# cheshmi/parsy_bench

Measured on AMD Instinct MI355X. Metric: Cholesky factorizations/sec (+ SpTRSV solves/sec), SuiteSparse SPD set, higher is better.
Workload: dtype f64; 1 GPU; flan-class stand-in (BASELINE.json configs[2] when flan: Flan_1565): grid (116, 116, 116) 27-point stencil, geometric nested dissection; n=1560896, nnz_A_lower=21491316, nsuper=81191, nnz_L=2044454227, xsize=2421483055, etree_levels=17, launches_per_factorization=357, parallelism=1 GPU

## Files before the change

### include/parsy_amd.h

```cpp
#ifndef PARSY_AMD_H
#define PARSY_AMD_H

#include <stdbool.h>
#include <stddef.h>
#include <stdint.h>

#ifdef __cplusplus
extern "C" {
#endif


bool cholesky_left_par_05(int n, int* c, int* r, double* values, size_t* lC, int* lR,
                          size_t* Li_ptr, double* lValues, int* blockSet, int supNo,
                          double* timing, int* aTree, int* cT, int* rT, int* col2Sup,
                          int nLevels, int* levelPtr, int* levelSet, int nPar, int* parPtr,
                          int* partition, int chunk, int threads, int super_max, int col_max,
                          double* nodCost);

bool cholesky_left_par_05_prune(int n, int* c, int* r, double* values, size_t* lC, int* lR,
                                size_t* Li_ptr, double* lValues, int* blockSet, int supNo,
                                double* timing, int* prunePtr, int* pruneSet, int nLevels,
                                int* levelPtr, int* levelSet, int nPar, int* parPtr, int* partition,
                                int chunk, int threads, int super_max, int col_max, double* nodCost);

bool cholesky_left_par_waveFront(int n, int* c, int* r, double* values, size_t* lC, int* lR,
                                 size_t* Li_ptr, double* lValues, int* blockSet, int supNo,
                                 double* timing, int* aTree, int* cT, int* rT, int* col2Sup,
                                 int nLevels, int* levelPtr, int* levelSet, int chunk,
                                 int threads, int super_max, int col_max);

int blockedLsolve(int n, size_t* Lp, int* Li, double* Lx, int NNZ, size_t* Li_ptr,
                  int* col2sup, int* sup2col, int supNo, double* x);
int leveledBlockedLsolve(int n, size_t* Lp, int* Li, double* Lx, int NNZ, size_t* Li_ptr,
                         int* col2sup, int* sup2col, int supNo, double* x, int levels,
                         int* levelPtr, int* levelSet, int chunk);
int H2LeveledBlockedLsolve(int n, size_t* Lp, int* Li, double* Lx, int NNZ, size_t* Li_ptr,
                           int* col2sup, int* sup2col, int supNo, double* x, int levels,
                           int* levelPtr, int* levelSet, int parts, int* parPtr,
                           int* partition, int chunk);
int H2LeveledBlockedLsolve_Peeled(int n, size_t* Lp, int* Li, double* Lx, int NNZ,
                                  size_t* Li_ptr, int* col2sup, int* sup2col, int supNo,
                                  double* x, int levels, int* levelPtr, int* levelSet,
                                  int parts, int* parPtr, int* partition, int chunk,
                                  int threads);

void parsy_dropin_reset(void);


typedef struct parsy_plan parsy_plan;

typedef struct parsy_plan_info {
    int32_t n, nsuper, nlevels, max_width, max_rows;
    int32_t n_small, n_big;
    int32_t chol_launches;
    int32_t solve_launches;
    int64_t nnzA, ssize, xsize, nnzL;
    int64_t n_updates;
    int64_t relpos_len;
    int64_t device_bytes;
    double flops_stored;
    double update_flops;
    double reread_bytes;
    double inner_flops;
    double tile_update_flops;
    double big_flops;
    int64_t big_entries;
    int32_t big_tasks;
    int32_t n_pieces;
    int32_t chol_levels;
    int32_t piece_width, big_min_k;
    int32_t chol_subtrees, chol_subtree_supernodes;
    int32_t solve_subtrees, solve_subtree_supernodes;
    int32_t backsolve_launches;
    int32_t dense_tasks;
    double dense_flops;
    int64_t dense_entries;
    int32_t solve_one;
    int32_t solve_one_blocks;
    int32_t sub_mrhs_trees;
    int32_t sub_mrhs_slots;
    int32_t sub_mrhs_tiers;
    int32_t sub_mrhs_cover_level;
    int64_t dense_strip_entries;
} parsy_plan_info;

parsy_plan* parsy_plan_create(int n, int supNo, const int* blockSet, const size_t* lC,
                              const size_t* Li_ptr, const int* lR, const int* aTree,
                              const int* col2Sup, const int* cT, const int* rT, const int* c,
                              const int* r, int device);
void parsy_plan_destroy(parsy_plan* plan);
int parsy_plan_get_info(const parsy_plan* plan, parsy_plan_info* info);

int parsy_plan_set_active(parsy_plan* plan, const uint8_t* mask);
long long parsy_plan_chain_check(const parsy_plan* plan, int slots);
long long parsy_plan_check(const parsy_plan* plan);

int parsy_factor_device(parsy_plan* plan, const double* d_values, double* d_lValues,
                        void* stream);
#define PARSY_FACTOR_NO_INIT 1
int parsy_factor_device_ex(parsy_plan* plan, const double* d_values, double* d_lValues,
                           void* stream, int flags);
int parsy_factor_status(parsy_plan* plan);

int parsy_factor_begin(parsy_plan* plan, const double* d_values, double* d_lValues, void* stream, int flags);
int parsy_factor_level(parsy_plan* plan, int level, double* d_lValues, void* stream);
int parsy_factor_end(parsy_plan* plan, void* stream);
int parsy_plan_pieces(const parsy_plan* plan, int32_t* supernode, int32_t* level, int32_t* col0, int32_t* width,
                      int32_t* rows, int64_t* value_begin, int64_t* value_end);
int parsy_plan_set_active_pieces(parsy_plan* plan, const uint8_t* piece_mask);

typedef struct parsy_dist parsy_dist;
typedef struct parsy_dist_info {
    int32_t nranks, nlevels, n_pieces, n_subtrees, n_root_pieces, n_messages;
    int64_t exchange_elements;
    double total_cost, root_cost;
    double max_rank_cost;
    double lockstep_cost;
} parsy_dist_info;
parsy_dist* parsy_dist_create(const parsy_plan* plan, int nranks, int block);
void parsy_dist_destroy(parsy_dist* dist);
int parsy_dist_get_info(const parsy_dist* dist, parsy_dist_info* info);
int parsy_dist_get(const parsy_dist* dist, int32_t* owner, uint8_t* in_subtree, double* rank_cost,
                   double* level_cost);
int parsy_dist_level_messages(const parsy_dist* dist, int level);
int parsy_dist_message(const parsy_dist* dist, int level, int index, int32_t* src, int32_t* dst, int64_t* nseg,
                       int64_t* total, const int64_t** off, const int32_t** len, const int64_t** packed);
long long parsy_dist_check(const parsy_plan* plan, const parsy_dist* dist);

int parsy_solve_device(parsy_plan* plan, const double* d_lValues, double* d_x, int nrhs,
                       int ldx, void* stream);

int parsy_solve_status(parsy_plan* plan);

int parsy_backsolve_device(parsy_plan* plan, const double* d_lValues, double* d_x, int nrhs, int ldx,
                           void* stream);
int parsy_plan_solve_levels(const parsy_plan* plan, int32_t* level);
#define PARSY_SOLVE_FIRST 1
#define PARSY_SOLVE_LAST 2
#define PARSY_SOLVE_BACKWARD 4
int parsy_solve_levels_device(parsy_plan* plan, const double* d_lValues, double* d_x, int nrhs, int ldx, void* stream,
                              int level_begin, int level_end, int flags);
int parsy_rhs_ones_device(parsy_plan* plan, const double* d_lValues, double* d_b, void* stream);
int parsy_copy_segments_device(double* d_dst, const double* d_src, const int64_t* d_dst_off,
                               const int64_t* d_src_off, const int32_t* d_len, int64_t nseg, void* stream);
int parsy_solve2_host(parsy_plan* plan, const double* lValues, double* x, int nrhs, int ldx,
                      int forward, double* seconds);

int parsy_plan_set_perm(parsy_plan* plan, const int* perm);
int parsy_residual_device(parsy_plan* plan, const double* d_values, const double* d_x, int ldx, const double* d_b,
                          int ldb, double* d_r, int ldr, int nrhs, double* berr, void* stream);
int parsy_solve_spd_device(parsy_plan* plan, const double* d_values, const double* d_lValues, const double* d_b,
                           int ldb, double* d_x, int ldx, int nrhs, int max_steps, int32_t* steps, double* berr,
                           void* stream);
int parsy_solve_spd_host(parsy_plan* plan, const double* values, const double* lValues, const double* b, int ldb,
                         double* x, int ldx, int nrhs, int max_steps, int32_t* steps, double* berr, double* seconds);

typedef struct parsy_selinv_info {
    int32_t levels;
    int32_t block_columns;
    int32_t tiled_block_columns;
    int32_t launches;
    double  flops;
    int64_t device_bytes;
} parsy_selinv_info;
int parsy_selinv_get_info(parsy_plan* plan, parsy_selinv_info* info);
long long parsy_selinv_check(const parsy_plan* plan);
int parsy_selinv_device(parsy_plan* plan, const double* d_lValues, double* d_z, void* stream);
int parsy_inverse_diag_device(parsy_plan* plan, const double* d_z, double* d_diag, void* stream);
int parsy_selinv_host(parsy_plan* plan, const double* lValues, double* z, double* diag, double* seconds);
int parsy_logdet_device(parsy_plan* plan, const double* d_lValues, double* logdet, void* stream);

int parsy_factor_host(parsy_plan* plan, const double* values, double* lValues, double* seconds);
int parsy_solve_host(parsy_plan* plan, const double* lValues, double* x, int nrhs, int ldx,
                     double* seconds);

double parsy_last_factor_ms(parsy_plan* plan);
double parsy_last_solve_ms(parsy_plan* plan);

#define PARSY_PROFILE_KINDS 10
int parsy_plan_profile(parsy_plan* plan, int enable);
int parsy_plan_profile_collect(parsy_plan* plan);
int parsy_plan_profile_get(parsy_plan* plan, double* kind_ms, int* kind_launches, int* runs);
int parsy_plan_profile_levels(parsy_plan* plan, double* main_ms, double* side_ms);

const char* parsy_last_error(void);

int parsy_device_count(void);

int parsy_debug_kernel_count(void);
const char* parsy_debug_kernel_name(int k);
unsigned long long parsy_debug_kernel_launches(int k);
void parsy_debug_kernel_reset(void);


typedef struct parsy_symbolic parsy_symbolic;

typedef struct parsy_symbolic_view {
    int32_t n, nsuper, nlevels, maxSupWid, maxCol;
    int64_t ssize, xsize, nnzL, nnzA, n_updates;
    double flops_colcount, flops_stored;
    const int* Perm;
    const int* Parent;
    const int* ColCount;
    const int* super;
    const int* col2Sup;
    const int* sParent;
    const size_t* p;
    const size_t* i_ptr;
    const int* s;
    const int* A1p; const int* A1i;
    const int* A2p; const int* A2i; const double* A2x;
    const int* A2src;
    const int* levelPtr;
    const int* levelSet;
    const int64_t* updPtr;
    const int* updSn; const int* updLb; const int* updUb;
} parsy_symbolic_view;

parsy_symbolic* parsy_analyze(int n, const int* Ap, const int* Ai, const double* Ax,
                              const int* perm, const int* nrelax, const double* zrelax);
void parsy_symbolic_free(parsy_symbolic* sym);
int parsy_symbolic_get(const parsy_symbolic* sym, parsy_symbolic_view* view);
parsy_plan* parsy_plan_from_symbolic(const parsy_symbolic* sym, int device);


int64_t parsy_grid_spd_lower(int nx, int ny, int nz, int stencil, double shift, int* Ap,
                             int* Ai, double* Ax);
int parsy_grid_nested_dissection(int nx, int ny, int nz, int leaf, int* perm);
int parsy_order_nd(int n, const int* Ap, const int* Ai, int leaf, int* perm);


typedef struct parsy_mg parsy_mg;
parsy_mg* parsy_mg_create(const parsy_symbolic* sym, int nranks, const int* devices, int block);
void parsy_mg_destroy(parsy_mg* mg);
int parsy_mg_set_values(parsy_mg* mg, const double* values);
int parsy_mg_factor(parsy_mg* mg, double* seconds);
int parsy_mg_profile(parsy_mg* mg, double* main_ms, double* side_ms, double* copy_ms);
int parsy_mg_rank_ms(parsy_mg* mg, double* rank_ms);
int parsy_mg_gather_host(parsy_mg* mg, double* lValues);
const parsy_dist* parsy_mg_dist(const parsy_mg* mg);
parsy_plan* parsy_mg_plan(parsy_mg* mg, int rank);

#ifdef __cplusplus
}
#endif
#endif
```

### parsy_bench_amd/_native.py

```python
from __future__ import annotations

import ctypes as C
import os
from pathlib import Path

import numpy as np

_PKG = Path(__file__).resolve().parent
_LIB_PATH = Path(os.environ["PARSY_LIB"]) if os.environ.get("PARSY_LIB") else _PKG / "libparsy_amd.so"
_lib = None

c_int_p = C.POINTER(C.c_int)
c_dbl_p = C.POINTER(C.c_double)
c_size_p = C.POINTER(C.c_size_t)
c_i64_p = C.POINTER(C.c_int64)


class SymbolicView(C.Structure):
    _fields_ = [
        ("n", C.c_int32), ("nsuper", C.c_int32), ("nlevels", C.c_int32),
        ("maxSupWid", C.c_int32), ("maxCol", C.c_int32),
        ("ssize", C.c_int64), ("xsize", C.c_int64), ("nnzL", C.c_int64),
        ("nnzA", C.c_int64), ("n_updates", C.c_int64),
        ("flops_colcount", C.c_double), ("flops_stored", C.c_double),
        ("Perm", c_int_p), ("Parent", c_int_p), ("ColCount", c_int_p),
        ("super", c_int_p), ("col2Sup", c_int_p), ("sParent", c_int_p),
        ("p", c_size_p), ("i_ptr", c_size_p), ("s", c_int_p),
        ("A1p", c_int_p), ("A1i", c_int_p),
        ("A2p", c_int_p), ("A2i", c_int_p), ("A2x", c_dbl_p), ("A2src", c_int_p),
        ("levelPtr", c_int_p), ("levelSet", c_int_p),
        ("updPtr", c_i64_p), ("updSn", c_int_p), ("updLb", c_int_p), ("updUb", c_int_p),
    ]


class PlanInfo(C.Structure):
    _fields_ = [
        ("n", C.c_int32), ("nsuper", C.c_int32), ("nlevels", C.c_int32),
        ("max_width", C.c_int32), ("max_rows", C.c_int32),
        ("n_small", C.c_int32), ("n_big", C.c_int32),
        ("chol_launches", C.c_int32), ("solve_launches", C.c_int32),
        ("nnzA", C.c_int64), ("ssize", C.c_int64), ("xsize", C.c_int64), ("nnzL", C.c_int64),
        ("n_updates", C.c_int64), ("relpos_len", C.c_int64), ("device_bytes", C.c_int64),
        ("flops_stored", C.c_double), ("update_flops", C.c_double), ("reread_bytes", C.c_double),
        ("inner_flops", C.c_double), ("tile_update_flops", C.c_double),
        ("big_flops", C.c_double), ("big_entries", C.c_int64), ("big_tasks", C.c_int32),
        ("n_pieces", C.c_int32), ("chol_levels", C.c_int32), ("piece_width", C.c_int32),
        ("big_min_k", C.c_int32),
        ("chol_subtrees", C.c_int32), ("chol_subtree_supernodes", C.c_int32),
        ("solve_subtrees", C.c_int32), ("solve_subtree_supernodes", C.c_int32),
        ("backsolve_launches", C.c_int32), ("dense_tasks", C.c_int32),
        ("dense_flops", C.c_double), ("dense_entries", C.c_int64),
        ("solve_one", C.c_int32), ("solve_one_blocks", C.c_int32),
        ("sub_mrhs_trees", C.c_int32), ("sub_mrhs_slots", C.c_int32),
        ("sub_mrhs_tiers", C.c_int32), ("sub_mrhs_cover_level", C.c_int32),
        ("dense_strip_entries", C.c_int64),
    ]

    def as_dict(self):
        return {k: getattr(self, k) for k, _ in self._fields_}


EXPORTED_SYMBOLS = [
    "cholesky_left_par_05", "cholesky_left_par_05_prune", "cholesky_left_par_waveFront", "blockedLsolve",
    "leveledBlockedLsolve", "H2LeveledBlockedLsolve", "H2LeveledBlockedLsolve_Peeled",
    "parsy_dropin_reset", "parsy_plan_create", "parsy_plan_destroy", "parsy_plan_get_info",
    "parsy_plan_set_active", "parsy_plan_chain_check", "parsy_factor_device", "parsy_factor_status", "parsy_solve_device",
    "parsy_factor_host", "parsy_solve_host", "parsy_last_factor_ms", "parsy_last_solve_ms",
    "parsy_last_error", "parsy_device_count", "parsy_analyze", "parsy_symbolic_free",
    "parsy_symbolic_get", "parsy_plan_from_symbolic", "parsy_grid_spd_lower",
    "parsy_grid_nested_dissection", "parsy_order_nd", "parsy_plan_profile", "parsy_plan_profile_collect",
    "parsy_plan_profile_get", "parsy_factor_device_ex", "parsy_backsolve_device", "parsy_solve_levels_device", "parsy_plan_solve_levels", "parsy_solve2_host",
    "parsy_rhs_ones_device", "parsy_solve_status", "parsy_copy_segments_device", "parsy_plan_check",
    "parsy_factor_begin", "parsy_factor_level", "parsy_factor_end", "parsy_plan_pieces",
    "parsy_plan_set_active_pieces", "parsy_dist_create", "parsy_dist_destroy", "parsy_dist_get_info",
    "parsy_dist_get", "parsy_dist_level_messages", "parsy_dist_message", "parsy_dist_check",
    "parsy_mg_create", "parsy_mg_destroy", "parsy_mg_set_values", "parsy_mg_factor", "parsy_mg_rank_ms",
    "parsy_mg_gather_host", "parsy_mg_dist", "parsy_mg_plan", "parsy_mg_profile", "parsy_plan_profile_levels",
    "parsy_debug_kernel_count", "parsy_debug_kernel_name", "parsy_debug_kernel_launches", "parsy_debug_kernel_reset",
    "parsy_plan_set_perm", "parsy_residual_device", "parsy_solve_spd_device", "parsy_solve_spd_host",
    "parsy_selinv_get_info", "parsy_selinv_check", "parsy_selinv_device", "parsy_inverse_diag_device",
    "parsy_selinv_host", "parsy_logdet_device",
]


class SelinvInfo(C.Structure):
    _fields_ = [
        ("levels", C.c_int32), ("block_columns", C.c_int32), ("tiled_block_columns", C.c_int32),
        ("launches", C.c_int32), ("flops", C.c_double), ("device_bytes", C.c_int64),
    ]

    def as_dict(self):
        return {k: getattr(self, k) for k, _ in self._fields_}


class DistInfo(C.Structure):
    _fields_ = [
        ("nranks", C.c_int32), ("nlevels", C.c_int32), ("n_pieces", C.c_int32), ("n_subtrees", C.c_int32),
        ("n_root_pieces", C.c_int32), ("n_messages", C.c_int32), ("exchange_elements", C.c_int64),
        ("total_cost", C.c_double), ("root_cost", C.c_double), ("max_rank_cost", C.c_double),
        ("lockstep_cost", C.c_double),
    ]

    def as_dict(self):
        return {k: getattr(self, k) for k, _ in self._fields_}


def _declare(lib):
    vp = C.c_void_p
    lib.parsy_last_error.restype = C.c_char_p
    lib.parsy_device_count.restype = C.c_int
    lib.parsy_debug_kernel_count.restype = C.c_int
    lib.parsy_debug_kernel_name.restype = C.c_char_p
    lib.parsy_debug_kernel_name.argtypes = [C.c_int]
    lib.parsy_debug_kernel_launches.restype = C.c_ulonglong
    lib.parsy_debug_kernel_launches.argtypes = [C.c_int]
    lib.parsy_debug_kernel_reset.restype = None
    lib.parsy_analyze.restype = vp
    lib.parsy_analyze.argtypes = [C.c_int, vp, vp, vp, vp, vp, vp]
    lib.parsy_symbolic_free.argtypes = [vp]
    lib.parsy_symbolic_get.argtypes = [vp, C.POINTER(SymbolicView)]
    lib.parsy_grid_spd_lower.restype = C.c_int64
    lib.parsy_grid_spd_lower.argtypes = [C.c_int, C.c_int, C.c_int, C.c_int, C.c_double, vp, vp, vp]
    lib.parsy_grid_nested_dissection.argtypes = [C.c_int, C.c_int, C.c_int, C.c_int, vp]
    lib.parsy_order_nd.argtypes = [C.c_int, vp, vp, C.c_int, vp]
    lib.parsy_plan_create.restype = vp
    lib.parsy_plan_create.argtypes = [C.c_int, C.c_int] + [vp] * 10 + [C.c_int]
    lib.parsy_plan_from_symbolic.restype = vp
    lib.parsy_plan_from_symbolic.argtypes = [vp, C.c_int]
    lib.parsy_plan_destroy.argtypes = [vp]
    lib.parsy_plan_get_info.argtypes = [vp, C.POINTER(PlanInfo)]
    lib.parsy_plan_set_active.argtypes = [vp, vp]
    lib.parsy_plan_chain_check.argtypes = [vp, C.c_int]
    lib.parsy_plan_chain_check.restype = C.c_longlong
    lib.parsy_plan_check.argtypes = [vp]
    lib.parsy_plan_check.restype = C.c_longlong
    lib.parsy_factor_device.argtypes = [vp, vp, vp, vp]
    lib.parsy_factor_device_ex.argtypes = [vp, vp, vp, vp, C.c_int]
    lib.parsy_factor_status.argtypes = [vp]
# ... 111 lines not shown
```

### parsy_bench_amd/api.py

```python
from __future__ import annotations

import ctypes as C

import numpy as np

from . import _native as N

KIND_NAMES = ["SMALL", "TILES", "CHAIN", "BIG", "BACK_BELOW", "SOLVE_SMALL", "SOLVE_PANEL", "SOLVE_FIXUP", "BACK_BLOCK", "DENSE"]


def device_count() -> int:
    return int(N.lib().parsy_device_count())


def kernel_launches() -> dict:
    lib = N.lib()
    return {lib.parsy_debug_kernel_name(k).decode(): int(lib.parsy_debug_kernel_launches(k))
            for k in range(lib.parsy_debug_kernel_count())}


def reset_kernel_launches() -> None:
    N.lib().parsy_debug_kernel_reset()


def _i32(a):
    return np.ascontiguousarray(a, dtype=np.int32)


def _sz(a):
    return np.ascontiguousarray(a, dtype=np.uint64)


def _f64(a):
    return np.ascontiguousarray(a, dtype=np.float64)


def cholesky_left_par_05(n, c, r, values, lC, lR, Li_ptr, lValues, blockSet, supNo, timing, aTree,
                         cT, rT, col2Sup, nLevels, levelPtr, levelSet, nPar, parPtr, partition,
                         chunk, threads, super_max, col_max, nodCost=None) -> bool:
    assert lValues.dtype == np.float64 and lValues.flags["C_CONTIGUOUS"]
    a = [_i32(c), _i32(r), _f64(values), _sz(lC), _i32(lR), _sz(Li_ptr), _i32(blockSet), _i32(aTree),
         _i32(cT), _i32(rT), _i32(col2Sup), _i32(levelPtr), _i32(parPtr), _i32(partition)]
    ls = None if levelSet is None else _i32(levelSet)
    return bool(N.lib().cholesky_left_par_05(
        n, N.ptr(a[0]), N.ptr(a[1]), N.ptr(a[2]), N.ptr(a[3]), N.ptr(a[4]), N.ptr(a[5]), N.ptr(lValues),
        N.ptr(a[6]), supNo, N.ptr(timing), N.ptr(a[7]), N.ptr(a[8]), N.ptr(a[9]), N.ptr(a[10]), nLevels,
        N.ptr(a[11]), N.ptr(ls), nPar, N.ptr(a[12]), N.ptr(a[13]), chunk, threads, super_max, col_max,
        None))


def cholesky_left_par_05_prune(n, c, r, values, lC, lR, Li_ptr, lValues, blockSet, supNo, timing, prunePtr,
                               pruneSet, nLevels, levelPtr, levelSet, nPar, parPtr, partition, chunk, threads,
                               super_max, col_max, nodCost=None) -> bool:
    assert lValues.dtype == np.float64 and lValues.flags["C_CONTIGUOUS"]
    a = [_i32(c), _i32(r), _f64(values), _sz(lC), _i32(lR), _sz(Li_ptr), _i32(blockSet), _i32(prunePtr),
         _i32(pruneSet), _i32(levelPtr), _i32(parPtr), _i32(partition)]
    ls = None if levelSet is None else _i32(levelSet)
    return bool(N.lib().cholesky_left_par_05_prune(
        n, N.ptr(a[0]), N.ptr(a[1]), N.ptr(a[2]), N.ptr(a[3]), N.ptr(a[4]), N.ptr(a[5]), N.ptr(lValues),
        N.ptr(a[6]), supNo, N.ptr(timing), N.ptr(a[7]), N.ptr(a[8]), nLevels, N.ptr(a[9]), N.ptr(ls), nPar,
        N.ptr(a[10]), N.ptr(a[11]), chunk, threads, super_max, col_max, None))


def cholesky_left_par_waveFront(n, c, r, values, lC, lR, Li_ptr, lValues, blockSet, supNo, timing,
                                aTree, cT, rT, col2Sup, nLevels, levelPtr, levelSet, chunk, threads,
                                super_max, col_max) -> bool:
    assert lValues.dtype == np.float64 and lValues.flags["C_CONTIGUOUS"]
    a = [_i32(c), _i32(r), _f64(values), _sz(lC), _i32(lR), _sz(Li_ptr), _i32(blockSet), _i32(aTree),
         _i32(cT), _i32(rT), _i32(col2Sup), _i32(levelPtr), _i32(levelSet)]
    return bool(N.lib().cholesky_left_par_waveFront(
        n, N.ptr(a[0]), N.ptr(a[1]), N.ptr(a[2]), N.ptr(a[3]), N.ptr(a[4]), N.ptr(a[5]), N.ptr(lValues),
        N.ptr(a[6]), supNo, N.ptr(timing), N.ptr(a[7]), N.ptr(a[8]), N.ptr(a[9]), N.ptr(a[10]), nLevels,
        N.ptr(a[11]), N.ptr(a[12]), chunk, threads, super_max, col_max))


def _solve_base(n, Lp, Li, Lx, NNZ, Li_ptr, col2sup, sup2col, supNo, x):
    assert x is None or (x.dtype == np.float64 and x.flags["C_CONTIGUOUS"])
    keep = [None if Lp is None else _sz(Lp), None if Li is None else _i32(Li), _f64(Lx), _sz(Li_ptr),
            _i32(col2sup), _i32(sup2col)]
    return keep, (n, N.ptr(keep[0]), N.ptr(keep[1]), N.ptr(keep[2]), int(NNZ), N.ptr(keep[3]),
                  N.ptr(keep[4]), N.ptr(keep[5]), supNo, N.ptr(x))


def blockedLsolve(n, Lp, Li, Lx, NNZ, Li_ptr, col2sup, sup2col, supNo, x) -> int:
    keep, base = _solve_base(n, Lp, Li, Lx, NNZ, Li_ptr, col2sup, sup2col, supNo, x)
    return int(N.lib().blockedLsolve(*base))


def leveledBlockedLsolve(n, Lp, Li, Lx, NNZ, Li_ptr, col2sup, sup2col, supNo, x, levels, levelPtr,
                         levelSet, chunk) -> int:
    keep, base = _solve_base(n, Lp, Li, Lx, NNZ, Li_ptr, col2sup, sup2col, supNo, x)
# ... 176 lines not shown
        if N.lib().parsy_selinv_device(self._h, d_lValues, d_z, stream) != 0:
            raise RuntimeError("parsy_selinv_device failed: " + N.last_error())

    def inverse_diag_device(self, d_z: int, d_diag: int, stream: int = 0) -> None:
        if N.lib().parsy_inverse_diag_device(self._h, d_z, d_diag, stream) != 0:
            raise RuntimeError("parsy_inverse_diag_device failed: " + N.last_error())

    def logdet_device(self, d_lValues: int, stream: int = 0):
        out = C.c_double(0)
        rc = N.lib().parsy_logdet_device(self._h, d_lValues, C.byref(out), stream)
        if rc < 0:
            raise RuntimeError("parsy_logdet_device failed: " + N.last_error())
        return out.value, int(rc)

    def backsolve_device(self, d_lValues: int, d_x: int, nrhs: int, ldx: int, stream: int = 0) -> None:
        if N.lib().parsy_backsolve_device(self._h, d_lValues, d_x, nrhs, ldx, stream) != 0:
            raise RuntimeError("parsy_backsolve_device failed: " + N.last_error())

    def rhs_ones_device(self, d_lValues: int, d_b: int, stream: int = 0) -> None:
        if N.lib().parsy_rhs_ones_device(self._h, d_lValues, d_b, stream) != 0:
            raise RuntimeError("parsy_rhs_ones_device failed: " + N.last_error())

    def factor_device(self, d_values: int, d_lValues: int, stream: int = 0, init: bool = True) -> None:
        if N.lib().parsy_factor_device_ex(self._h, d_values, d_lValues, stream, 0 if init else 1) != 0:
            raise RuntimeError("parsy_factor_device failed: " + N.last_error())

    def solve_device(self, d_lValues: int, d_x: int, nrhs: int, ldx: int, stream: int = 0) -> None:
        if N.lib().parsy_solve_device(self._h, d_lValues, d_x, nrhs, ldx, stream) != 0:
            raise RuntimeError("parsy_solve_device failed: " + N.last_error())

    def solve_levels(self) -> np.ndarray:
        out = np.zeros(self.sym.nsuper, dtype=np.int32)
        N.lib().parsy_plan_solve_levels(self._h, N.ptr(out))
        return out

    def solve_levels_device(self, d_lValues: int, d_x: int, nrhs: int, ldx: int, stream: int, level_begin: int, level_end: int,
                            first: bool, last: bool, backward: bool = False) -> None:
        flags = (1 if first else 0) | (2 if last else 0) | (4 if backward else 0)
        if N.lib().parsy_solve_levels_device(self._h, d_lValues, d_x, nrhs, ldx, stream, level_begin, level_end, flags) != 0:
            raise RuntimeError("parsy_solve_levels_device failed: " + N.last_error())

    def factor_begin(self, d_values: int, d_lValues: int, stream: int = 0, init: bool = True) -> None:
        if N.lib().parsy_factor_begin(self._h, d_values, d_lValues, stream, 0 if init else 1) != 0:
            raise RuntimeError("parsy_factor_begin failed: " + N.last_error())

    def factor_level(self, level: int, d_lValues: int, stream: int = 0) -> None:
        if N.lib().parsy_factor_level(self._h, level, d_lValues, stream) != 0:
            raise RuntimeError("parsy_factor_level failed: " + N.last_error())

    def factor_end(self, stream: int = 0) -> None:
        if N.lib().parsy_factor_end(self._h, stream) != 0:
            raise RuntimeError("parsy_factor_end failed: " + N.last_error())

    def pieces(self) -> dict:
        n = int(N.lib().parsy_plan_pieces(self._h, *([None] * 7)))
        out = {k: np.zeros(n, dtype=np.int32) for k in ("supernode", "level", "col0", "width", "rows")}
        out.update({k: np.zeros(n, dtype=np.int64) for k in ("value_begin", "value_end")})
        N.lib().parsy_plan_pieces(self._h, *[N.ptr(out[k]) for k in (
            "supernode", "level", "col0", "width", "rows", "value_begin", "value_end")])
        return out

    def set_active_pieces(self, mask) -> None:
        m = None if mask is None else np.ascontiguousarray(mask, dtype=np.uint8)
        if N.lib().parsy_plan_set_active_pieces(self._h, N.ptr(m)) != 0:
            raise RuntimeError(N.last_error())

    def check(self) -> int:
        return int(N.lib().parsy_plan_check(self._h))

    def last_factor_ms(self) -> float:
        return float(N.lib().parsy_last_factor_ms(self._h))

    def last_solve_ms(self) -> float:
        return float(N.lib().parsy_last_solve_ms(self._h))

    def profile(self, mode: int) -> None:
        N.lib().parsy_plan_profile(self._h, mode)

    def profile_collect(self) -> None:
        if N.lib().parsy_plan_profile_collect(self._h) != 0:
            raise RuntimeError("profile_collect: no profiled run to collect")

    def profile_get(self) -> dict:
        ms = np.zeros(10, dtype=np.float64)
        cnt = np.zeros(10, dtype=np.int32)
        runs = C.c_int(0)
        N.lib().parsy_plan_profile_get(self._h, N.ptr(ms), N.ptr(cnt), C.byref(runs))
        return {"runs": runs.value, "ms": dict(zip(KIND_NAMES, ms.tolist())),
                "launches": dict(zip(KIND_NAMES, cnt.tolist()))}


class Dist:

    def __init__(self, plan: "Plan", nranks: int, block: int = 0, _borrowed=None):
        self._own = _borrowed is None
        self._h = _borrowed or N.lib().parsy_dist_create(plan._h, nranks, block)
        if not self._h:
            raise RuntimeError("parsy_dist_create failed: " + N.last_error())
        di = N.DistInfo()
        N.lib().parsy_dist_get_info(self._h, C.byref(di))
        self.info = di.as_dict()
        self.nranks, self.nlevels = di.nranks, di.nlevels
        self.owner = np.zeros(di.n_pieces, dtype=np.int32)
        self.in_subtree = np.zeros(di.n_pieces, dtype=np.uint8)
        self.rank_cost = np.zeros(di.nranks)
        self.level_cost = np.zeros((di.nlevels, di.nranks))
        N.lib().parsy_dist_get(self._h, N.ptr(self.owner), N.ptr(self.in_subtree), N.ptr(self.rank_cost),
                               N.ptr(self.level_cost))

    def close(self):
        h, self._h = self._h, None
        if h and self._own:
            N.lib().parsy_dist_destroy(h)

    def __del__(self):
        try:
            self.close()
        except Exception:
            pass

    def check(self, plan: "Plan") -> int:
        return int(N.lib().parsy_dist_check(plan._h, self._h))

    def mask(self, rank: int) -> np.ndarray:
        return (self.owner == rank).astype(np.uint8)

    def messages(self, level: int, rank: int | None = None):
        lib = N.lib()
        out = []
        for k in range(max(int(lib.parsy_dist_level_messages(self._h, level)), 0)):
            src, dst = C.c_int32(0), C.c_int32(0)
            nseg, total = C.c_int64(0), C.c_int64(0)
            if lib.parsy_dist_message(self._h, level, k, C.byref(src), C.byref(dst), C.byref(nseg), C.byref(total),
                                      None, None, None) != 0:
                raise RuntimeError(N.last_error())
            if rank is not None and rank not in (src.value, dst.value):
                continue
            off, ln, pk = N.c_i64_p(), N.c_int_p(), N.c_i64_p()
            lib.parsy_dist_message(self._h, level, k, None, None, None, None, C.byref(off), C.byref(ln), C.byref(pk))
            out.append((src.value, dst.value, N.view_array(off, nseg.value, np.int64),
                        N.view_array(ln, nseg.value, np.int32), N.view_array(pk, nseg.value, np.int64), total.value))
        return out


class MultiDevice:

    def __init__(self, sym, devices, block: int = 0):
        if not getattr(sym, "_handle", None):
            raise RuntimeError("MultiDevice needs an inspector result (parsy_symbolic)")
        dv = np.ascontiguousarray(devices, dtype=np.int32)
        self.sym = sym
        self.nranks = len(dv)
        self._h = N.lib().parsy_mg_create(sym._handle, len(dv), N.ptr(dv), block)
        if not self._h:
            raise RuntimeError("parsy_mg_create failed: " + N.last_error())
        self.dist = Dist(None, len(dv), _borrowed=N.lib().parsy_mg_dist(self._h))

    def close(self):
        h, self._h = self._h, None
        if h:
            self.dist._h = None
            N.lib().parsy_mg_destroy(h)

    def __del__(self):
        try:
            self.close()
        except Exception:
            pass
# ... 32 lines not shown
```

### parsy_bench_amd/csrc/capi_exec.hip

```cpp
#include <hip/hip_runtime.h>

#include <chrono>
#include <cstdio>
#include <cstring>
#include <map>
#include <algorithm>
#include <atomic>
#include <mutex>
#include <thread>
#include <string>
#include <tuple>
#include <vector>

#include "../../include/parsy_amd.h"
#include "errors.hpp"
#include "dist.hpp"
#include "executor.hpp"
#include "inspector.hpp"
#include "refine.hpp"

using parsy::set_last_error;

namespace {

// ... 230 lines not shown
        set_last_error("parsy_plan_create: null or negative argument");
        return nullptr;
    }
    if (device >= 0 && device >= parsy_device_count()) {
        set_last_error("parsy_plan_create: no usable HIP device " + std::to_string(device) +
                       " (this library has no CPU fallback; pass device < 0 for a host-only schedule)");
        return nullptr;
    }
    parsy::PatternRef P;
    P.n = n;
    P.nsuper = supNo;
    P.super = blockSet;
    P.col2sup = col2Sup;
    P.sparent = aTree;
    P.i_ptr = Li_ptr;
    P.s = lR;
    P.A1p = cT;
    P.A1i = rT;
    return parsy::plan_build(P, lC, c, r, device);
}

parsy_plan* parsy_plan_from_symbolic(const parsy_symbolic* sym, int device) {
    const parsy::Symbolic* S = parsy_symbolic_cxx(sym);
    if (!S) {
        set_last_error("parsy_plan_from_symbolic: null symbolic");
        return nullptr;
    }
    return parsy_plan_create(S->n, S->nsuper, S->super.data(), S->p.data(), S->i_ptr.data(), S->s.data(),
                             S->sparent.data(), S->col2sup.data(), S->A1.p.data(), S->A1.i.data(),
                             S->A2.p.data(), S->A2.i.data(), device);
}

void parsy_plan_destroy(parsy_plan* plan) { parsy::plan_free(plan); }

int parsy_plan_get_info(const parsy_plan* pl, parsy_plan_info* o) {
    if (!pl || !o) return -1;
    const parsy::Schedule& S = pl->S;
    std::memset(o, 0, sizeof(*o));
    o->n = S.n;
    o->nsuper = S.nsuper;
    o->nlevels = S.nlevels;
    o->max_width = S.max_width;
    o->max_rows = S.max_rows;
    o->n_small = S.n_small;
    o->n_big = S.n_big;
    o->chol_launches = (int32_t)S.chol.size() + 1;
    o->solve_launches = (int32_t)S.solve.size();
    o->nnzA = S.nnzA;
    o->ssize = S.ssize;
    o->xsize = S.xsize;
    o->nnzL = S.nnzL;
    o->n_updates = (int64_t)S.upd.size();
    o->relpos_len = (int64_t)S.relpos.size();
    o->device_bytes = pl->device_bytes;
    o->flops_stored = S.flops_stored;
    o->update_flops = S.update_flops;
    o->reread_bytes = S.reread_bytes;
    o->inner_flops = S.inner_flops;
    o->tile_update_flops = S.tile_update_flops;
    o->big_flops = S.big_flops;
    o->big_entries = (int64_t)S.big_entries.size();
    o->big_tasks = (int32_t)S.big_tasks.size();
    o->n_pieces = (int32_t)S.csn.size();
    o->chol_levels = S.cnlevels;
    o->piece_width = S.piece_width;
    o->big_min_k = S.big_min_k;
    o->chol_subtrees = (int32_t)S.small_ranges.size() / 2;
    for (size_t b = 0; b + 1 < S.small_ranges.size(); b += 2) o->chol_subtree_supernodes += S.small_ranges[b + 1] - S.small_ranges[b];
    o->solve_subtrees = (int32_t)S.solve_small_ranges.size() / 2;
    for (size_t b = 0; b + 1 < S.solve_small_ranges.size(); b += 2)
        o->solve_subtree_supernodes += S.solve_small_ranges[b + 1] - S.solve_small_ranges[b];
    o->backsolve_launches = (int32_t)S.bsolve.size();
    for (const parsy::Launch& l : S.chol)
        if (l.kind == parsy::kLaunchDense) o->dense_tasks += l.count;
    o->dense_flops = S.dense_flops;
    o->dense_entries = S.n_dense_entries;
    o->solve_one = (S.solve_one ? 1 : 0) | (S.solve_one_back ? 2 : 0) | ((S.solve_one || S.solve_one_back) && S.one_subtrees ? 4 : 0);
    o->solve_one_blocks = S.solve_one ? (int32_t)S.one_f.sn.size() : S.solve_one_back ? (int32_t)S.one_back().sn.size() : 0;
    o->sub_mrhs_trees = (int32_t)S.sub_trees.size();
    o->sub_mrhs_slots = S.sub_max_slots;
    o->sub_mrhs_tiers = (int32_t)S.sub_tiers.size();
    o->sub_mrhs_cover_level = S.sub_cover_level;
    o->dense_strip_entries = S.n_strip_entries;
    return 0;
}

long long parsy_plan_chain_check(const parsy_plan* pl, int slots) {
    if (!pl || slots < 1) {
        set_last_error("parsy_plan_chain_check: null plan or slots < 1");
        return -1;
    }
    return (long long)simulate_chain(pl->S, slots);
}

long long parsy_plan_check(const parsy_plan* pl) {
    if (!pl) {
        set_last_error("parsy_plan_check: null plan");
        return -1;
    }
    std::string what;
    const long long bad = (long long)parsy::check_schedule(pl->S, what);
    if (bad) set_last_error("parsy_plan_check: " + what);
    return bad;
}

int parsy_plan_set_active(parsy_plan* pl, const uint8_t* mask) {
    if (!pl) return -1;
    std::vector<uint8_t> pieces;
    if (pl->piece_mask_set) pieces = pl->S.active_piece;
    parsy::build_launches(pl->S, mask, pl->piece_mask_set ? pieces.data() : nullptr);
    pl->sn_mask_set = mask != nullptr;
    return parsy::plan_upload_launches(pl);
}

int parsy_plan_set_active_pieces(parsy_plan* pl, const uint8_t* piece_mask) {
    if (!pl) return -1;
    std::vector<uint8_t> sn_mask;
    if (pl->sn_mask_set) sn_mask = pl->S.active;
    parsy::build_launches(pl->S, pl->sn_mask_set ? sn_mask.data() : nullptr, piece_mask);
    pl->piece_mask_set = piece_mask != nullptr;
    return parsy::plan_upload_launches(pl);
}

int parsy_plan_pieces(const parsy_plan* pl, int32_t* supernode, int32_t* level, int32_t* col0, int32_t* width,
                      int32_t* rows, int64_t* value_begin, int64_t* value_end) {
    if (!pl) return -1;
    const parsy::Schedule& S = pl->S;
    const int nc = (int)S.csn.size();
    for (int p = 0; p < nc; ++p) {
        const parsy::SnDesc& C = S.csn[(size_t)p];
        const parsy::SnDesc& R = S.sn[(size_t)S.csn_real[(size_t)p]];
        if (supernode) supernode[p] = S.csn_real[(size_t)p];
        if (level) level[p] = S.level_of.empty() ? 0 : S.level_of[(size_t)p];
        if (col0) col0[p] = C.c0;
        if (width) width[p] = C.w;
        if (rows) rows[p] = C.r;
        if (value_begin) value_begin[p] = R.px + (int64_t)C.rbias * R.r;
        if (value_end) value_end[p] = R.px + (int64_t)(C.rbias + C.w) * R.r;
    }
    return nc;
}

int parsy_plan_solve_levels(const parsy_plan* pl, int32_t* level) {
    if (!pl) return -1;
    const parsy::Schedule& S = pl->S;
    if (level)
        for (int l = 0; l < S.nlevels; ++l)
            for (int q = S.levelPtr[(size_t)l]; q < S.levelPtr[(size_t)l + 1]; ++q) level[S.levelSet[(size_t)q]] = l;
    return S.nlevels;
}

int64_t parsy_debug_big_entries(const parsy_plan* pl, int32_t* out, int64_t cap) {
    if (!pl) return -1;
    const parsy::Schedule& S = pl->S;
    int64_t n = 0, t = 0;
    for (const parsy::Schedule::BigTask& b : S.big_all) {
        for (int64_t e = b.e0; e < b.e1; ++e, ++n) {
            if (!out || n >= cap) continue;
            const parsy::WaveEntry& E = S.big_entries[(size_t)e];
            int32_t* o = out + 7 * n;
            o[0] = (int32_t)t;
            o[1] = b.src_level * 2 + (b.next ? 0 : 1);
            o[2] = E.K;
            o[3] = E.mn & 255;
            o[4] = (E.mn >> 8) & 255;
            o[5] = ((E.mn >> 16) & 1) != 0;
// ... 64 lines not shown
    }
    return parsy::plan_factor_begin(pl, d_values, d_lValues, (hipStream_t)stream, (flags & PARSY_FACTOR_NO_INIT) == 0);
}

int parsy_factor_level(parsy_plan* pl, int level, double* d_lValues, void* stream) {
    if (!pl || !d_lValues) {
        set_last_error("parsy_factor_level: null argument");
        return -1;
    }
    return parsy::plan_factor_levels(pl, level, level + 1, d_lValues, (hipStream_t)stream);
}

int parsy_factor_end(parsy_plan* pl, void* stream) {
    if (!pl) {
        set_last_error("parsy_factor_end: null plan");
        return -1;
    }
    return parsy::plan_factor_end(pl, (hipStream_t)stream);
}

int parsy_factor_device(parsy_plan* pl, const double* d_values, double* d_lValues, void* stream) {
    if (!pl || !d_values || !d_lValues) {
        set_last_error("parsy_factor_device: null argument");
        return -1;
    }
    return parsy::plan_factor(pl, d_values, d_lValues, (hipStream_t)stream);
}

int parsy_factor_device_ex(parsy_plan* pl, const double* d_values, double* d_lValues, void* stream,
                           int flags) {
    if (!pl || !d_values || !d_lValues) {
        set_last_error("parsy_factor_device_ex: null argument");
        return -1;
    }
    return parsy::plan_factor(pl, d_values, d_lValues, (hipStream_t)stream,
                              (flags & PARSY_FACTOR_NO_INIT) == 0);
}

int parsy_factor_status(parsy_plan* pl) {
    if (!pl || pl->device < 0) return -1;
    int v = 0;
    if (hipMemcpy(&v, pl->dp.info, sizeof(int), hipMemcpyDeviceToHost) != hipSuccess) return -1;
    return v >= 0x7f7f7f7f ? 0 : v;
}

int parsy_solve_status(parsy_plan* pl) {
    if (!pl || pl->device < 0) return -1;
    int v = 0;
    const int* word = pl->solve_status_word ? pl->solve_status_word : pl->dp.sinfo;
    if (hipMemcpy(&v, word, sizeof(int), hipMemcpyDeviceToHost) != hipSuccess) return -1;
    if (v < 0) set_last_error("solve: a hand-off wait inside a chain launch timed out; x is not the solution");
    return v < 0 ? -1 : 0;
}

int parsy_solve_device(parsy_plan* pl, const double* d_lValues, double* d_x, int nrhs, int ldx,
                       void* stream) {
    if (!pl || !d_lValues || !d_x) {
        set_last_error("parsy_solve_device: null argument");
        return -1;
    }
    return parsy::plan_solve(pl, d_lValues, d_x, nrhs, ldx, (hipStream_t)stream);
}

double parsy_last_factor_ms(parsy_plan* pl) {
    float ms = -1;
    if (!pl || !pl->have_f) return -1;
    if (hipEventSynchronize(pl->ev_f1) != hipSuccess) return -1;
    if (hipEventElapsedTime(&ms, pl->ev_f0, pl->ev_f1) != hipSuccess) return -1;
    return ms;
}

double parsy_last_solve_ms(parsy_plan* pl) {
    float ms = -1;
    if (!pl || !pl->have_s) return -1;
    if (hipEventSynchronize(pl->ev_s1) != hipSuccess) return -1;
    if (hipEventElapsedTime(&ms, pl->ev_s0, pl->ev_s1) != hipSuccess) return -1;
    return ms;
}

int parsy_plan_profile(parsy_plan* pl, int enable) {
    if (!pl) return -1;
    pl->profile = enable != 0;
    if (enable == 2) {
        for (int k = 0; k < 10; ++k) pl->kind_ms[k] = 0, pl->kind_launches[k] = 0;
        pl->profiled_runs = 0;
        pl->level_ms.clear();
    }
    return 0;
}

int parsy_plan_profile_collect(parsy_plan* pl) { return pl ? parsy::plan_collect_profile(pl) : -1; }

int parsy_plan_profile_get(parsy_plan* pl, double* kind_ms, int* kind_launches, int* runs) {
    if (!pl) return -1;
    for (int k = 0; k < 10; ++k) {
        if (kind_ms) kind_ms[k] = pl->kind_ms[k];
        if (kind_launches) kind_launches[k] = pl->kind_launches[k];
    }
    if (runs) *runs = pl->profiled_runs;
    return 0;
}

int parsy_plan_profile_levels(parsy_plan* pl, double* main_ms, double* side_ms) {
    if (!pl) return -1;
    const int nl = pl->S.cnlevels;
    for (int l = 0; l < nl; ++l) {
        const size_t a = (size_t)l << 1, b = a | 1;
        if (main_ms) main_ms[l] = a < pl->level_ms.size() ? pl->level_ms[a] : 0.0;
        if (side_ms) side_ms[l] = b < pl->level_ms.size() ? pl->level_ms[b] : 0.0;
    }
    return nl;
}

static void build_download_bands(parsy_plan* pl) {
    const parsy::Schedule& S = pl->S;
    const int nl = S.cnlevels, np = (int)S.csn.size();
    {
        std::vector<double> bytes((size_t)nl, 0.0);
        for (int p = 0; p < np; ++p) bytes[(size_t)S.level_of[(size_t)p]] += 8.0 * S.csn[(size_t)p].w * S.csn[(size_t)p].ld;
        const double total = 8.0 * (double)S.xsize;
        pl->h_band_level.clear();
        double run = 0, next = total / 8;
        for (int l = 0; l < nl; ++l) {
            run += bytes[(size_t)l];
            if (l == nl - 1 || run >= next) {
                pl->h_band_level.push_back(l);
                while (next <= run) next += total / 8;
            }
        }
    }
    const size_t nb = pl->h_band_level.size();
    pl->h_band_runs.assign(nb, {});
    std::vector<int> band_of((size_t)nl, 0);
    for (size_t b = 0, l = 0; b < nb; ++b)
        for (; (int)l <= pl->h_band_level[b]; ++l) band_of[l] = (int)b;
    const int64_t gap = 131072;
    for (int p = 0; p < np; ++p) {
        const parsy::SnDesc& C = S.csn[(size_t)p];
        const parsy::SnDesc& R = S.sn[(size_t)S.csn_real[(size_t)p]];
        const int64_t a = R.px + (int64_t)C.rbias * R.r, e = R.px + (int64_t)(C.rbias + C.w) * R.r;
        auto& runs = pl->h_band_runs[(size_t)band_of[(size_t)S.level_of[(size_t)p]]];
        if (!runs.empty() && a - (runs.back().first + runs.back().second) <= gap && a >= runs.back().first)
            runs.back().second = std::max(runs.back().second, e - runs.back().first);
        else
            runs.push_back({a, e - a});
    }
}

int parsy_factor_host(parsy_plan* pl, const double* values, double* lValues, double* seconds) {
    if (!pl || !values || !lValues) {
        set_last_error("parsy_factor_host: null argument");
        return -1;
    }
    if (pl->device < 0) {
        set_last_error("parsy_factor_host: plan has no device");
        return -1;
    }
    const parsy::Schedule& S = pl->S;
    CAPI_HIP(hipSetDevice(pl->device), -1);
    if (!pl->h_values_dev) CAPI_HIP(hipMalloc((void**)&pl->h_values_dev, std::max<int64_t>(S.nnzA, 1) * 8), -1);
    if (!pl->h_L_dev) CAPI_HIP(hipMalloc((void**)&pl->h_L_dev, std::max<int64_t>(S.xsize, 1) * 8), -1);
    CAPI_HIP(hipMemcpy(pl->h_values_dev, values, (size_t)S.nnzA * 8, hipMemcpyHostToDevice), -1);
    const char* pe = std::getenv("PARSY_HOST_PIPELINE");
    const bool pipeline_on = !(pe && pe[0] == '0'), pipeline_forced = pe && pe[0] == '2';
    if (!pipeline_on || (!pipeline_forced && S.xsize * 8 < (int64_t)256 << 20) || pl->profile || S.cnlevels < 1) {
        if (parsy::plan_factor(pl, pl->h_values_dev, pl->h_L_dev, nullptr) != 0) return -1;
        CAPI_HIP(hipDeviceSynchronize(), -1);
        if (seconds) *seconds = parsy_last_factor_ms(pl) * 1e-3;
        CAPI_HIP(hipMemcpy(lValues, pl->h_L_dev, (size_t)S.xsize * 8, hipMemcpyDeviceToHost), -1);
        return 0;
    }
    if (!pl->h_ready) {
        hipStream_t hs = nullptr, hc = nullptr;
        std::vector<hipEvent_t> evs;
        auto undo = [&] {
            for (hipEvent_t e : evs) (void)hipEventDestroy(e);
            if (hs) (void)hipStreamDestroy(hs);
            if (hc) (void)hipStreamDestroy(hc);
// ... 408 lines not shown
```

### parsy_bench_amd/csrc/chol_kernels.hip

```cpp
#include <hip/hip_runtime.h>

#include <algorithm>

#include <climits>

#include "kernels.hpp"

namespace parsy {

typedef double double4_t __attribute__((ext_vector_type(4)));

static constexpr int kThreads = 256;
static constexpr int kLdSub = kSub + 1;
static constexpr int kLdDiag = kTile + 1;

#ifdef PARSY_BIGSTAMPS
__device__ unsigned long long g_bigtrace[2 * 8 * 1024];
__device__ int g_bigstamp_cfg[2];
#define BIGSTAMP(i) do { if (st_on) g_bigtrace[((size_t)st_slot * 1024 + st_n) * 8 + (i)] = __builtin_readcyclecounter(); } while (0)
#else
#define BIGSTAMP(i) do { } while (0)
#endif

#ifdef PARSY_STAMPS
__device__ unsigned long long g_stamps[32];
#define STAMP(i) do { if (threadIdx.x == 0) g_stamps[i] = wall_clock64(); } while (0)
__device__ unsigned long long g_trace[16 * 512];
__device__ unsigned long long g_probe[8];
#define TRACE(J, i) do { if (threadIdx.x == 0 && (J) < 512) g_trace[(J) * 16 + (i)] = wall_clock64(); } while (0)
__device__ unsigned long long g_tilephase[16];
#define TPHASE(i) do { if (threadIdx.x == 0) { const unsigned long long now_ = wall_clock64(); \
                       atomicAdd(&g_tilephase[i], now_ - tp_last); tp_last = now_; } } while (0)
#else
#define STAMP(i) do { } while (0)
#define TRACE(J, i) do { } while (0)
#define TPHASE(i) do { } while (0)
#endif

__global__ __launch_bounds__(kThreads) void k_scatter_a(const double* __restrict__ values,
                                                        const int64_t* __restrict__ a_dst,
                                                        double* __restrict__ L, int64_t nnz) {
    for (int64_t q = (int64_t)blockIdx.x * kThreads + threadIdx.x; q < nnz;
         q += (int64_t)gridDim.x * kThreads)
        L[a_dst[q]] = values[q];
}

void launch_scatter_a(const double* values, const int64_t* a_dst, double* L, int64_t nnz,
                      hipStream_t stream) {
    if (nnz <= 0) return;
    int64_t blocks = (nnz + kThreads - 1) / kThreads;
    if (blocks > 4096) blocks = 4096;
    hipLaunchKernelGGL(k_scatter_a, dim3((unsigned)blocks), dim3(kThreads), 0, stream, values, a_dst,
                       L, nnz);
}

typedef double double2_t __attribute__((ext_vector_type(2)));
typedef __attribute__((address_space(3))) double lds_f64;
static constexpr int kPotrfScratch = 2 * 4 * kTile;
__device__ __forceinline__ double readlane_f64(double v, int src_lane) {
    return __hiloint2double(__builtin_amdgcn_readlane(__double2hiint(v), src_lane),
                            __builtin_amdgcn_readlane(__double2loint(v), src_lane));
}
__device__ __forceinline__ void potrf64_regs(double (&a)[4][4], double* __restrict__ scr, int ti, int tj,
                                             int nb, int& bad, double* __restrict__ inv_out = nullptr) {
    const bool lower = ti >= tj;
    bad = 0;
#ifdef PARSY_STAMPS
#define PPROBE(i) do { if (tjj == 4 && ti == 6 && tj == 4) g_probe[i] = clock64(); } while (0)
#else
#define PPROBE(i) do { } while (0)
#endif
    const int nsteps = (nb + 3) / 4;
    for (int tjj = 0; tjj < nsteps; ++tjj) {
        double2_t* __restrict__ pub = reinterpret_cast<double2_t*>(scr) + (tjj & 1) * (2 * kTile);
        PPROBE(0);
        if ((tj >> 2) == (tjj >> 2)) {
            const int src = __builtin_amdgcn_readfirstlane((tjj & 3) * 16 + tjj);
            double l[4][4], inv[4];
            int nonpos = 0;
#pragma unroll
            for (int jj = 0; jj < 4; ++jj) {
                double d = readlane_f64(a[jj][jj], src);
#pragma unroll
                for (int k = 0; k < jj; ++k) d = fma(-l[jj][k], l[jj][k], d);
                nonpos |= (d > 0.0) ? 0 : (1 << jj);
                const double y0 = __builtin_amdgcn_rsq(d);
                const double e = fma(-d * y0, y0, 1.0);
                inv[jj] = fma(y0 * e, fma(e, 0.375, 0.5), y0);
                l[jj][jj] = d * inv[jj];
#pragma unroll
                for (int ii = jj + 1; ii < 4; ++ii) {
                    double v = readlane_f64(a[ii][jj], src);
#pragma unroll
                    for (int k = 0; k < jj; ++k) v = fma(-l[ii][k], l[jj][k], v);
                    l[ii][jj] = v * inv[jj];
                }
            }
            PPROBE(1);
            if (nonpos && bad == 0 && tj == tjj && lower) {
                const int jj = __builtin_ctz(nonpos);
                if (4 * tjj + jj < nb) bad = 4 * tjj + jj + 1;
            }
            if (tj == tjj && lower) {
                if (ti == tjj) {
#pragma unroll
                    for (int ri = 0; ri < 4; ++ri)
#pragma unroll
                        for (int ci = 0; ci <= ri; ++ci) a[ri][ci] = l[ri][ci];
                    if (inv_out) {
#pragma unroll
                        for (int jj = 0; jj < 4; ++jj) inv_out[4 * tjj + jj] = (4 * tjj + jj < nb) ? inv[jj] : 1.0;
                    }
                } else {
#pragma unroll
                    for (int ri = 0; ri < 4; ++ri)
#pragma unroll
                        for (int jj = 0; jj < 4; ++jj) {
                            double v = a[ri][jj];
#pragma unroll
                            for (int k = 0; k < jj; ++k) v = fma(-a[ri][k], l[jj][k], v);
                            a[ri][jj] = v * inv[jj];
                        }
                }
#pragma unroll
                for (int ci = 0; ci < 4; ++ci)
#pragma unroll
                    for (int h = 0; h < 2; ++h) pub[(2 * ci + h) * 16 + ti] = double2_t{a[2 * h][ci], a[2 * h + 1][ci]};
            }
        }
        PPROBE(2);
        __syncthreads();
        PPROBE(3);
        if (lower && tj > tjj) {
            double li[4][4], lc[4][4];
#pragma unroll
            for (int k = 0; k < 4; ++k)
// ... 2119 lines not shown
```

### parsy_bench_amd/csrc/executor.hip

```cpp
#include "executor.hpp"

#include <climits>
#include <cstdlib>
#include <cstring>
#include <stdexcept>

#include "errors.hpp"
#include "plan_fwd.hpp"
#include "refine.hpp"
#include "selinv.hpp"

namespace parsy {

const Schedule& plan_schedule(const parsy_plan* plan) { return plan->S; }

#define PARSY_HIP(call)                                                                      \
    do {                                                                                     \
        hipError_t e_ = (call);                                                              \
        if (e_ != hipSuccess) {                                                              \
            set_last_error(std::string(#call) + ": " + hipGetErrorString(e_));               \
            return -1;                                                                       \
        }                                                                                    \
    } while (0)

// ... 7 lines not shown
    if (!v.empty()) PARSY_HIP(hipMemcpy(d, v.data(), v.size() * sizeof(T), hipMemcpyHostToDevice));
    pl->device_bytes += (int64_t)bytes;
    dptr = (const T*)d;
    return 0;
}

int plan_upload_launches(parsy_plan* pl) {
    if (pl->device < 0) return 0;
    PARSY_HIP(hipSetDevice(pl->device));
    for (void* d : pl->launch_owned) (void)hipFree(d);
    pl->launch_owned.clear();
    pl->levels_open = false;
    const Schedule& S = pl->S;
    if (upload(pl, S.small_list, pl->dp.small_list, true)) return -1;
    if (upload(pl, S.small_ranges, pl->dp.small_ranges, true)) return -1;
    if (upload(pl, S.solve_small_ranges, pl->dp.solve_small_ranges, true)) return -1;
    if (upload(pl, S.bsolve_ranges, pl->dp.bsolve_ranges, true)) return -1;
    if (upload(pl, S.tiles, pl->dp.tiles, true)) return -1;
    if (upload(pl, S.big_tasks, pl->dp.big_tasks, true)) return -1;
    if (upload(pl, S.solve_small_list, pl->dp.solve_small_list, true)) return -1;
    if (upload(pl, S.solve_panels, pl->dp.solve_panels, true)) return -1;
    if (upload(pl, S.solve_mtasks, pl->dp.solve_mtasks, true)) return -1;
    if (upload(pl, S.solve_fix_list, pl->dp.solve_fix_list, true)) return -1;
    if (upload(pl, S.solve_wide_list, pl->dp.solve_wide_list, true)) return -1;
    if (upload(pl, S.bsolve_blocks, pl->dp.bsolve_blocks, true)) return -1;
    if (upload(pl, S.bsolve_below, pl->dp.bsolve_below, true)) return -1;
    if (pl->dp.bpart) {
        (void)hipFree(pl->dp.bpart);
        pl->dp.bpart = nullptr;
    }
    if (upload(pl, S.bsolve_pairs, pl->dp.bsolve_pairs, true)) return -1;
    if (upload(pl, S.sub_members, pl->dp.sub_members, true) || upload(pl, S.sub_trees, pl->dp.sub_trees, true) ||
        upload(pl, S.sub_slots, pl->dp.sub_slots, true) || upload(pl, S.sub_out_rows, pl->dp.sub_out_rows, true))
        return -1;
    pl->dp.sub_ntiers = (!S.sub_tiers.empty() && solve_sub_prepare(S.sub_max_slots) == 0) ? (int)S.sub_tiers.size() : 0;
    {
        auto up = [&](const Schedule::OneLists& O, DevicePattern::OneDev& D) {
            D = DevicePattern::OneDev();
            if (upload(pl, O.sn, D.sn, true) || upload(pl, O.slot0, D.slot0, true) || upload(pl, O.wleft, D.wleft, true) ||
                upload(pl, O.pull_ptr, D.pull_ptr, true) || upload(pl, O.pull_slot, D.pull_slot, true) ||
                upload(pl, O.pull_pos, D.pull_pos, true))
                return -1;
            D.nblocks = (int)O.sn.size();
            D.nslots = std::max<int64_t>(O.nslots, 1);
            return 0;
        };
        if (up(S.one_f, pl->dp.one_f)) return -1;
        if (S.one_b.sn.empty()) pl->dp.one_b = pl->dp.one_f;
        else if (up(S.one_b, pl->dp.one_b)) return -1;
        for (int d = 0; d < 2; ++d) {
            if (pl->one_y[d]) {
                (void)hipFree(pl->one_y[d]);
                pl->device_bytes -= pl->one_bytes[d];
            }
            pl->one_y[d] = nullptr;
            pl->one_bytes[d] = 0;
            pl->one_cap[d] = 0;
            pl->one_calls[d] = 0;
        }
        pl->solve_status_word = nullptr;
    }
    {
        void* d = nullptr;
        PARSY_HIP(hipMalloc(&d, (size_t)std::max(S.n_chain_launches, 1) * sizeof(int)));
        pl->launch_owned.push_back(d);
        pl->dp.tickets = (int*)d;
        PARSY_HIP(hipMalloc(&d, (size_t)std::max(S.n_solve_chain_launches, 1) * sizeof(int)));
        pl->launch_owned.push_back(d);
        pl->dp.stickets = (int*)d;
    }
    PARSY_HIP(hipDeviceSynchronize());
    return 0;
}

static int plan_upload(parsy_plan* pl) {
    PARSY_HIP(hipSetDevice(pl->device));
    const Schedule& S = pl->S;
    if (upload(pl, S.sn, pl->dp.sn, false)) return -1;
    if (upload(pl, S.csn, pl->dp.csn, false)) return -1;
    if (upload(pl, S.big_entries, pl->dp.big_entries, false)) return -1;
    if (upload(pl, S.upd, pl->dp.upd, false)) return -1;
    if (upload(pl, S.relpos, pl->dp.relpos, false)) return -1;
    if (upload(pl, S.a_dst, pl->dp.a_dst, false)) return -1;
    if (upload(pl, S.rows, pl->dp.rows, false)) return -1;
    if (upload(pl, S.wave_entries, pl->dp.wave_entries, false)) return -1;
    if (upload(pl, S.wave_ptr, pl->dp.wave_ptr, false)) return -1;
    if (upload(pl, S.split_ranges, pl->dp.split_ranges, false)) return -1;
    {
        void* d = nullptr;
        const size_t sbytes = (size_t)std::max<int64_t>(S.n_split_doubles, 1) * sizeof(double);
        PARSY_HIP(hipMalloc(&d, sbytes));
        pl->owned.push_back(d);
        pl->dp.tile_scratch = (double*)d;
        pl->device_bytes += (int64_t)sbytes;
    }
    {
        void* d = nullptr;
        PARSY_HIP(hipMalloc(&d, sizeof(int)));
        pl->owned.push_back(d);
        pl->dp.info = (int*)d;
        PARSY_HIP(hipMemset(d, 0x7f, sizeof(int)));
        PARSY_HIP(hipMalloc(&d, sizeof(int)));
        pl->owned.push_back(d);
        pl->dp.sinfo = (int*)d;
        PARSY_HIP(hipMemset(d, 0, sizeof(int)));
        const size_t tbytes = 2 * std::max<int64_t>(S.n_tflags, 1) * sizeof(int);
        pl->dp.n_tflags = (int)S.n_tflags;
        PARSY_HIP(hipMalloc(&d, tbytes));
        pl->owned.push_back(d);
        pl->dp.tflags = (int*)d;
        PARSY_HIP(hipMemset(d, 0, tbytes));
        pl->device_bytes += (int64_t)tbytes;
    }
    {
        int prio_least = 0, prio_greatest = 0;
        PARSY_HIP(hipDeviceGetStreamPriorityRange(&prio_least, &prio_greatest));
        PARSY_HIP(hipStreamCreateWithPriority(&pl->side_stream, hipStreamNonBlocking, prio_least));
    }
    PARSY_HIP(hipEventCreateWithFlags(&pl->ev_init, hipEventDisableTiming));
    pl->ev_level_done.resize(std::max(S.nlevels, S.cnlevels) + 1);
    pl->ev_early_done.resize(std::max(S.nlevels, S.cnlevels) + 1);
    for (auto& e : pl->ev_level_done) PARSY_HIP(hipEventCreateWithFlags(&e, hipEventDisableTiming));
    for (auto& e : pl->ev_early_done) PARSY_HIP(hipEventCreateWithFlags(&e, hipEventDisableTiming));
    {
        const char* no = std::getenv("PARSY_NO_OVERLAP");
        pl->overlap = !(no && no[0] == '1');
    }
    PARSY_HIP(hipEventCreate(&pl->ev_f0));
    PARSY_HIP(hipEventCreate(&pl->ev_f1));
    PARSY_HIP(hipEventCreate(&pl->ev_s0));
    PARSY_HIP(hipEventCreate(&pl->ev_s1));
    return plan_upload_launches(pl);
}

parsy_plan* plan_build(const PatternRef& P, const size_t* lC, const int* A2p, const int* A2i,
                       int device) {
    parsy_plan* pl = new parsy_plan;
    int cus = 0;
    if (device >= 0) {
        hipDeviceProp_t prop;
        if (hipGetDeviceProperties(&prop, device) == hipSuccess) cus = prop.multiProcessorCount;
        (void)hipSetDevice(device);
        const int per_cu = chain_workgroups_per_cu();
        if (per_cu == 1) cus = cus / 2;
    }
    try {
        build_schedule(P, lC, A2p, A2i, nullptr, pl->S, cus);
    } catch (const std::exception& e) {
        set_last_error(std::string("plan: ") + e.what());
        delete pl;
        return nullptr;
    }
    pl->solve_only = pl->S.solve_only;
    pl->device = device;
    if (device >= 0 && plan_upload(pl) != 0) {
        plan_free(pl);
        return nullptr;
    }
    return pl;
}

void plan_free(parsy_plan* pl) {
    if (!pl) return;
    if (pl->device >= 0) {
        (void)hipSetDevice(pl->device);
        (void)hipDeviceSynchronize();
        for (void* d : pl->owned) (void)hipFree(d);
        for (void* d : pl->launch_owned) (void)hipFree(d);
        if (pl->xscratch) (void)hipFree(pl->xscratch);
        for (double*& q : pl->one_y) {
            if (q) (void)hipFree(q);
            q = nullptr;
        }
        if (pl->xt) (void)hipFree(pl->xt);
        if (pl->dinv) (void)hipFree(pl->dinv);
        if (pl->dp.bpart) (void)hipFree(pl->dp.bpart);
        if (pl->h_values_dev) (void)hipFree(pl->h_values_dev);
        if (pl->h_L_dev) (void)hipFree(pl->h_L_dev);
        if (pl->h_x_dev) (void)hipFree(pl->h_x_dev);
        for (hipEvent_t e : {pl->ev_f0, pl->ev_f1, pl->ev_s0, pl->ev_s1})
            if (e) (void)hipEventDestroy(e);
        for (hipEvent_t e : pl->pev) (void)hipEventDestroy(e);
        for (hipEvent_t e : pl->ev_level_done) (void)hipEventDestroy(e);
        for (hipEvent_t e : pl->ev_early_done) (void)hipEventDestroy(e);
        if (pl->ev_init) (void)hipEventDestroy(pl->ev_init);
        if (pl->side_stream) (void)hipStreamDestroy(pl->side_stream);
        if (pl->h_stream) (void)hipStreamDestroy(pl->h_stream);
        if (pl->h_copy) (void)hipStreamDestroy(pl->h_copy);
        for (hipEvent_t e : pl->h_band_ev) (void)hipEventDestroy(e);
    }
    refine_free(pl);
    selinv_free(pl);
    delete pl;
}

static void profile_mark(parsy_plan* pl, int kind, hipStream_t stream, size_t& cursor, int level = -1, int side = 0,
                         int count = 0) {
    if (!pl->profile) return;
    if (cursor >= pl->pev_count.size()) pl->pev_count.resize(cursor + 1, 0);
    pl->pev_count[cursor] = count;
    if (cursor >= pl->pev_level.size()) pl->pev_level.resize(cursor + 1, 0);
    pl->pev_level[cursor] = level >= 0 ? (level << 1) | (side & 1) : -1;
    if (cursor >= pl->pev.size()) {
        hipEvent_t e;
        (void)hipEventCreate(&e);
        pl->pev.push_back(e);
    }
    if (cursor >= pl->pev_kind.size()) pl->pev_kind.push_back(kind);
    else pl->pev_kind[cursor] = kind;
    (void)hipEventRecord(pl->pev[cursor], stream);
    ++cursor;
}

static bool sub_tiers_usable(const parsy_plan* pl, int nrhs, int ldx) {
    const int m = pl->dp.gates.sub_mrhs_min;
    return pl->dp.sub_ntiers > 0 && m > 0 && nrhs >= m && ldx < (1 << 24) && nrhs < (1 << 20);
}

static void run_begin(parsy_plan* pl) {
    pl->run_cursor = 0;
    pl->run_next_level_event = 0;
    pl->run_early_seen.assign(pl->ev_early_done.size(), 0);
}

static void run_range(parsy_plan* pl, const std::vector<Launch>& seq, size_t i0, size_t i1, double* L,
                      const double* Lc, double* x, int nrhs, int ldx, hipStream_t stream) {
    size_t& cursor = pl->run_cursor;
    const bool overlap = pl->overlap && !pl->profile && pl->side_stream != nullptr;
    int& next_level_event = pl->run_next_level_event;
    std::vector<char>& early_seen = pl->run_early_seen;
    auto record_levels_below = [&](int level) {
        for (; next_level_event < level && next_level_event < (int)pl->ev_level_done.size(); ++next_level_event)
            (void)hipEventRecord(pl->ev_level_done[next_level_event], stream);
    };
    for (size_t li = i0; li < i1; ++li) {
        const Launch& l = seq[li];
        const bool on_side = overlap && l.side;
        if (!on_side) {
            if (overlap && is_chol_launch(l.kind)) record_levels_below(l.level);
            if (overlap && (l.kind == kLaunchChain || l.kind == kLaunchBig || l.kind == kLaunchDense)) {
                int lw = std::min<int>(l.level, (int)early_seen.size() - 1);
                while (lw >= 0 && !early_seen[lw]) --lw;
                if (lw >= 0) (void)hipStreamWaitEvent(stream, pl->ev_early_done[lw], 0);
            }
        }
        profile_mark(pl, l.kind, stream, cursor, l.level, l.side, l.count);
        switch (l.kind) {
            case kLaunchSmall: launch_chol_small(pl->dp, l.first, l.count, l.lds_bytes, l.jb, l.fused == 2, L, stream); break;
            case kLaunchTiles:
            case kLaunchBig:
            case kLaunchDense:
                if (on_side) {
                    record_levels_below(l.wait_level + 1);
                    (void)hipStreamWaitEvent(pl->side_stream,
                                             l.wait_level >= 0 ? pl->ev_level_done[l.wait_level] : pl->ev_init, 0);
                    if (l.kind == kLaunchBig) launch_chol_big(pl->dp, l.first, l.count, L, pl->side_stream);
                    else if (l.kind == kLaunchDense) launch_chol_dense(pl->dp, l.first, l.count, L, pl->side_stream);
                    else launch_chol_tiles(pl->dp, l.first, l.count, L, pl->side_stream);
                    (void)hipEventRecord(pl->ev_early_done[l.level], pl->side_stream);
                    early_seen[l.level] = 1;
                } else if (l.kind == kLaunchBig) {
                    launch_chol_big(pl->dp, l.first, l.count, L, stream);
                } else if (l.kind == kLaunchDense) {
                    launch_chol_dense(pl->dp, l.first, l.count, L, stream);
                } else {
                    launch_chol_tiles(pl->dp, l.first, l.count, L, stream);
                }
                break;
            case kLaunchChain: launch_chol_chain(pl->dp, l.first, l.count, l.jb, pl->epoch, l.fused != 0, L, stream); break;
            case kLaunchSolveSmall:
                if (l.fused == 2 && sub_tiers_usable(pl, nrhs, ldx) && pl->S.sub_tiers[0].ntrees == l.count)
                    launch_solve_sub_mrhs(pl->dp, pl->S.sub_tiers[0], Lc, x, nrhs, ldx, pl->solve_ldq, stream);
                else
                    launch_solve_small(pl->dp, l.first, l.count, l.jb, l.fused == 2, Lc, x, nrhs, ldx, pl->solve_ldq, stream);
                break;
            case kLaunchSolvePanel:
                if (l.fused && nrhs >= pl->dp.gates.chain_mrhs_min)
                    launch_solve_blocks_mrhs(pl->dp, l.lds_bytes, l.wait_level, Lc, pl->dinv, x, pl->xscratch, nrhs, ldx,
                                             pl->solve_ldq, l.jb, pl->dp.gates.wait_bias, stream);
                else if (l.fused)
                    launch_solve_chain(pl->dp, l.first, l.count, Lc, pl->dinv, x, pl->xscratch, l.jb, pl->dp.gates.wait_bias,
                                       stream);
                else
                    launch_solve_panel(pl->dp, l.first, l.count, Lc, x, pl->xscratch, nrhs, ldx, stream);
                break;
            case kLaunchSolveFixup:
                launch_solve_fixup(pl->dp, l.first, l.count, x, pl->xscratch, nrhs, ldx, stream);
                break;
            case kLaunchBackBelow:
                if (nrhs == 1) launch_bsolve_below(pl->dp, l.first, l.count, Lc, x, stream);
                break;
            case kLaunchBackBlock:
                if (l.fused == 1 && nrhs == 1) {
                    launch_bsolve_chain_w(pl->dp, l.lds_bytes, l.wait_level, Lc, pl->dinv, x, pl->xscratch, l.jb,
                                          pl->dp.gates.wait_bias, stream);
                    break;
                }
                if (l.fused == 2 && sub_tiers_usable(pl, nrhs, ldx) && pl->S.sub_tiers[0].ntrees == l.count) {
                    launch_bsolve_sub_mrhs(pl->dp, pl->S.sub_tiers[0], Lc, x, nrhs, ldx, stream);
                    break;
                }
                launch_bsolve_block(pl->dp, l.first, l.count, Lc, pl->dinv, x, pl->xscratch, nrhs, ldx, l.fused,
                                    l.early,
                                    l.fused == 1 ? l.jb : 0, pl->dp.gates.wait_bias, stream);
                break;
        }
    }
}

static void run_end(parsy_plan* pl, hipStream_t stream) {
    profile_mark(pl, -1, stream, pl->run_cursor);
    if (pl->profile) pl->pev_kind.resize(pl->run_cursor);
}

static void run_launches(parsy_plan* pl, const std::vector<Launch>& seq, double* L, const double* Lc,
                         double* x, int nrhs, int ldx, hipStream_t stream) {
    run_begin(pl);
    run_range(pl, seq, 0, seq.size(), L, Lc, x, nrhs, ldx, stream);
    run_end(pl, stream);
}
// ... 114 lines not shown
        for (size_t k = S.sub_tiers.size(); k-- > 0;) {
            profile_mark(pl, kLaunchBackBlock, stream, pl->run_cursor, 0, 0, S.sub_tiers[k].ntrees);
            launch_bsolve_sub_mrhs(pl->dp, S.sub_tiers[k], d_L, x, nrhs, ldx, stream);
        }
    }
    run_end(pl, stream);
}

static int solve_end(parsy_plan* pl, hipStream_t stream) {
    PARSY_HIP(hipGetLastError());
    PARSY_HIP(hipEventRecord(pl->ev_s1, stream));
    pl->have_s = true;
    return 0;
}

int plan_backsolve(parsy_plan* pl, const double* d_L, double* d_x, int nrhs, int ldx, hipStream_t stream) {
    if (solve_start(pl, "parsy_backsolve", nrhs >= 1 && ldx >= pl->S.n, "nrhs >= 1 and ldx >= n") != 0) return -1;
    const Schedule& S = pl->S;
    double *y = nullptr, *y_next = nullptr;
    int *st = nullptr, *st_next = nullptr;
    int one_rc = solve_takes_one_launch(pl, nrhs, true) ? one_begin(pl, true, nrhs, stream, y, y_next, st, st_next) : 1;
    if (one_rc < 0) return -1;
    if (one_rc == 0) {
        PARSY_HIP(hipEventRecord(pl->ev_s0, stream));
        run_begin(pl);
        profile_mark(pl, kLaunchBackBlock, stream, pl->run_cursor, 0, 0, pl->dp.one_b.nblocks);
        launch_bsolve_one(pl->dp, S.n, d_L, d_x, nrhs, ldx, y, y_next, st, st_next, pl->dp.gates.wait_bias, pl->one_cap[1],
                          stream);
        if (S.one_subtrees && S.n_bsolve_subtrees > 0)
            run_range(pl, S.bsolve, S.bsolve.size() - 1, S.bsolve.size(), nullptr, d_L, d_x, nrhs, ldx, stream);
        run_end(pl, stream);
        return solve_end(pl, stream);
    }
    const int64_t need = (int64_t)ldx * nrhs;
    const bool wide = !S.solve_wide_list.empty();
    if (solve_prologue(pl, d_L, nrhs, ldx, 0, S.max_width > kTile ? need : 0, true, nrhs > 1 && wide, wide ? need : 0,
                       stream) != 0)
        return -1;
    run_solve(pl, true, d_L, d_x, nrhs, ldx, stream);
    return solve_end(pl, stream);
}

int plan_solve_levels(parsy_plan* pl, const double* d_L, double* d_x, int nrhs, int ldx, hipStream_t stream, int lev0,
                      int lev1, int flags) {
    const bool first = flags & 1, last = flags & 2, backward = flags & 4;
    if (solve_start(pl, "parsy_solve_levels", nrhs >= 1 && ldx >= pl->S.n && lev0 <= lev1,
                    "nrhs >= 1, ldx >= n and level_begin <= level_end", first) != 0)
        return -1;
    if (!first && (!pl->levels_open || pl->levels_backward != backward || pl->levels_nrhs != nrhs)) {
        set_last_error("parsy_solve_levels: a step without PARSY_SOLVE_FIRST needs an open solve of the same direction and width");
        return -1;
    }
    const Schedule& S = pl->S;
    if (first) {
        const int64_t need = (int64_t)ldx * nrhs;
        const int64_t armed = S.n_solve_wide == 0 ? 0 : (!backward && nrhs == 1) ? (int64_t)ldx : need;
        if (solve_prologue(pl, d_L, nrhs, ldx, 0, (S.n_solve_wide > 0 || S.max_width > kTile) ? need : 0, backward, false,
                           armed, stream) != 0)
            return -1;
        pl->solve_ldq = 0;
        run_begin(pl);
        pl->levels_open = true;
        pl->levels_backward = backward;
        pl->levels_nrhs = nrhs;
    }
    const std::vector<Launch>& seq = backward ? S.bsolve : S.solve;
    for (size_t li = 0; li < seq.size(); ++li)
        if ((seq[li].level >= lev0 && seq[li].level < lev1) || (last && seq[li].kind == kLaunchSolveFixup))
            run_range(pl, seq, li, li + 1, nullptr, d_L, d_x, nrhs, ldx, stream);
    if (!last) return 0;
    run_end(pl, stream);
    pl->levels_open = false;
    return solve_end(pl, stream);
}

int plan_collect_profile(parsy_plan* pl) {
    if (!pl->profile || pl->pev_kind.size() < 2) return -1;
    for (size_t i = 0; i + 1 < pl->pev_kind.size(); ++i) {
        float ms = 0;
        if (hipEventElapsedTime(&ms, pl->pev[i], pl->pev[i + 1]) != hipSuccess) return -1;
        const int k = pl->pev_kind[i];
        if (pl->pev_ms.size() <= i) pl->pev_ms.resize(i + 1, 0.f);
        pl->pev_ms[i] = ms;
        if (k >= 0 && k < 10) {
            pl->kind_ms[k] += ms;
            pl->kind_launches[k] += 1;
        }
        if (is_chol_launch(k) && i < pl->pev_level.size() && pl->pev_level[i] >= 0) {
            const size_t slot = (size_t)pl->pev_level[i];
            if (pl->level_ms.size() <= slot) pl->level_ms.resize(slot + 1, 0.0);
            pl->level_ms[slot] += ms;
        }
    }
    pl->profiled_runs += 1;
    return 0;
}

int plan_factor_begin(parsy_plan* pl, const double* d_values, double* d_L, hipStream_t stream, bool init) {
    if (pl->device < 0) {
        set_last_error("parsy_factor: plan was built without a device (device < 0)");
        return -1;
    }
    if (pl->solve_only) {
        set_last_error("parsy_factor: plan was built from L's pattern only (solve-only)");
        return -1;
    }
    const Schedule& S = pl->S;
    if (pl->epoch >= INT_MAX - 4) {
        PARSY_HIP(hipMemsetAsync(pl->dp.tflags, 0, 2 * (size_t)std::max(pl->dp.n_tflags, 1) * sizeof(int), stream));
        pl->epoch = 0;
    }
    pl->epoch += 1;
    PARSY_HIP(hipEventRecord(pl->ev_f0, stream));
    if (init) PARSY_HIP(hipMemsetAsync(d_L, 0, (size_t)S.xsize * sizeof(double), stream));
    PARSY_HIP(hipMemsetAsync(pl->dp.info, 0x7f, sizeof(int), stream));
    PARSY_HIP(hipMemsetAsync(pl->dp.tickets, 0, (size_t)std::max(S.n_chain_launches, 1) * sizeof(int), stream));
    if (init) launch_scatter_a(d_values, pl->dp.a_dst, d_L, S.nnzA, stream);
    PARSY_HIP(hipEventRecord(pl->ev_init, stream));
    run_begin(pl);
    pl->factor_open = true;
    pl->factor_next_level = 0;
    return 0;
}

int plan_factor_levels(parsy_plan* pl, int level0, int level1, double* d_L, hipStream_t stream) {
    const Schedule& S = pl->S;
    if (!pl->factor_open) {
        set_last_error("parsy_factor_level: no factorization is open (call parsy_factor_begin first)");
        return -1;
    }
    if (level0 != pl->factor_next_level || level1 < level0 || level1 > S.cnlevels) {
        set_last_error("parsy_factor_level: levels must be enqueued in ascending order without gaps");
        return -1;
    }
    if (level1 > level0)
        run_range(pl, S.chol, S.chol_level_begin[(size_t)level0], S.chol_level_begin[(size_t)level1], d_L, d_L, nullptr,
                  0, 0, stream);
    profile_mark(pl, -1, stream, pl->run_cursor);
    pl->factor_next_level = level1;
    PARSY_HIP(hipGetLastError());
    return 0;
}

int plan_factor_end(parsy_plan* pl, hipStream_t stream) {
    if (!pl->factor_open) {
        set_last_error("parsy_factor_end: no factorization is open");
        return -1;
    }
    if (pl->factor_next_level != pl->S.cnlevels) {
        set_last_error("parsy_factor_end: not every level has been enqueued");
        return -1;
    }
    run_end(pl, stream);
    if (pl->overlap && !pl->profile && pl->side_stream != nullptr) {
        for (size_t k = pl->run_early_seen.size(); k-- > 0;)
            if (pl->run_early_seen[k]) {
                (void)hipStreamWaitEvent(stream, pl->ev_early_done[k], 0);
                break;
            }
    }
    PARSY_HIP(hipGetLastError());
    PARSY_HIP(hipEventRecord(pl->ev_f1, stream));
    pl->have_f = true;
    pl->factor_open = false;
    return 0;
}

void plan_factor_abort(parsy_plan* pl, hipStream_t stream) {
    if (!pl) return;
    (void)hipStreamSynchronize(stream);
    if (pl->side_stream != nullptr) (void)hipStreamSynchronize(pl->side_stream);
    (void)hipGetLastError();
    if (pl->factor_open) run_end(pl, stream);
    pl->factor_open = false;
    pl->factor_next_level = 0;
}

int plan_factor(parsy_plan* pl, const double* d_values, double* d_L, hipStream_t stream, bool init) {
    if (plan_factor_begin(pl, d_values, d_L, stream, init) != 0) return -1;
    if (plan_factor_levels(pl, 0, pl->S.cnlevels, d_L, stream) != 0) return -1;
    return plan_factor_end(pl, stream);
}

int plan_solve(parsy_plan* pl, const double* d_L, double* d_x, int nrhs, int ldx, hipStream_t stream) {
    if (solve_start(pl, "parsy_solve", nrhs >= 1 && ldx >= pl->S.n, "nrhs >= 1 and ldx >= n") != 0) return -1;
    const Schedule& S = pl->S;
    const SolveGates& G = pl->dp.gates;
    double *y = nullptr, *y_next = nullptr;
    int *st = nullptr, *st_next = nullptr;
    int one_rc = solve_takes_one_launch(pl, nrhs, false) ? one_begin(pl, false, nrhs, stream, y, y_next, st, st_next) : 1;
    if (one_rc < 0) return -1;
    if (one_rc == 0) {
        PARSY_HIP(hipEventRecord(pl->ev_s0, stream));
        run_begin(pl);
        pl->solve_ldq = 0;
        if (S.one_subtrees && S.n_solve_subtrees > 0) run_range(pl, S.solve, 0, 1, nullptr, d_L, d_x, nrhs, ldx, stream);
        profile_mark(pl, kLaunchSolveSmall, stream, pl->run_cursor, 0, 0, pl->dp.one_f.nblocks);
        launch_solve_one(pl->dp, d_L, d_x, nrhs, ldx, y, y_next, st, st_next, G.wait_bias, pl->one_cap[0], stream);
        run_end(pl, stream);
        return solve_end(pl, stream);
    }
    const bool use_xt = G.xt_min > 0 && nrhs >= G.xt_min && nrhs >= G.mrhs_min && S.solve_fix_list.empty() &&
                        (S.xsize >= (int64_t)150 * S.n || G.xt_min_set);
    const int ldq = use_xt ? (nrhs + 15) & ~15 : 0;
    const int64_t need = use_xt ? (int64_t)S.n * ldq : (int64_t)ldx * nrhs;
    if (use_xt) PARSY_HIP(grow_device(pl->xt, pl->xt_len, need));
    const bool arm_wide = nrhs >= G.chain_mrhs_min && S.n_solve_wide > 0 && !S.solve_wide_list.empty() &&
                          S.solve_fix_list.empty();
    const int64_t scratch = S.n_solve_wide > 0 ? need : 0;
    if (solve_prologue(pl, d_L, nrhs, ldx, ldq, scratch, false, arm_wide, scratch, stream) != 0) return -1;
    pl->solve_ldq = ldq;
    if (use_xt) launch_transpose_x(d_x, ldx, pl->xt, ldq, S.n, nrhs, true, stream);
    run_solve(pl, false, d_L, use_xt ? pl->xt : d_x, nrhs, ldx, stream);
    if (use_xt) launch_transpose_x(d_x, ldx, pl->xt, ldq, S.n, nrhs, false, stream);
    pl->solve_ldq = 0;
    return solve_end(pl, stream);
}

hipError_t grow_device(double*& buf, int64_t& len, int64_t need) {
    if (len >= need) return hipSuccess;
    if (buf) {
        const hipError_t e = hipFree(buf);
        if (e != hipSuccess) return e;
    }
    buf = nullptr;
    len = 0;
    const hipError_t e = hipMalloc((void**)&buf, (size_t)need * sizeof(double));
    if (e == hipSuccess) len = need;
    return e;
}

}
```

### parsy_bench_amd/csrc/executor.hpp

```cpp
#pragma once
#include <hip/hip_runtime.h>

#include <cstdint>
#include <mutex>
#include <string>
#include <vector>

#include "kernels.hpp"
#include "schedule.hpp"

namespace parsy {
struct RefineState;
struct SelinvState;
}

struct parsy_plan {
    parsy::Schedule S;
    int device = -1;
    std::mutex use_mu;
    bool solve_only = false;
    bool sn_mask_set = false, piece_mask_set = false;

    std::vector<void*> owned;
    std::vector<void*> launch_owned;
    parsy::DevicePattern dp;
    int64_t device_bytes = 0;
    int epoch = 0;

    double* dinv = nullptr;
    double* xscratch = nullptr;
    int64_t xscratch_len = 0;
    double* one_y[2] = {nullptr, nullptr};
    unsigned one_calls[2] = {0, 0};
    int one_cap[2] = {0, 0};
    int64_t one_bytes[2] = {0, 0};
    bool one_off = false, one_off_back = false;
    const int* solve_status_word = nullptr;

    double* h_values_dev = nullptr;
    double* h_L_dev = nullptr;
    double* h_x_dev = nullptr;
    hipStream_t h_stream = nullptr, h_copy = nullptr;
    std::vector<hipEvent_t> h_band_ev;
    bool h_ready = false;
    bool levels_open = false, levels_backward = false;
    int levels_nrhs = 0;
    std::vector<int> h_band_level;
    std::vector<std::vector<std::pair<int64_t, int64_t>>> h_band_runs;
    int64_t h_x_len = 0;

    hipStream_t side_stream = nullptr;
    hipEvent_t ev_init = nullptr;
    std::vector<hipEvent_t> ev_level_done, ev_early_done;
    bool overlap = true;

    size_t run_cursor = 0;
    int run_next_level_event = 0;
    std::vector<char> run_early_seen;
    bool factor_open = false;
    int factor_next_level = 0;

    hipEvent_t ev_f0 = nullptr, ev_f1 = nullptr, ev_s0 = nullptr, ev_s1 = nullptr;
    bool have_f = false, have_s = false;

    bool profile = false;
    double* xt = nullptr;
    int64_t xt_len = 0;
    int solve_ldq = 0;
    std::vector<hipEvent_t> pev;
    std::vector<int> pev_kind;
    std::vector<int> pev_level;
    std::vector<int> pev_count;
    std::vector<float> pev_ms;
    std::vector<double> level_ms;
    double kind_ms[10] = {0, 0, 0, 0, 0, 0, 0, 0, 0, 0};
    int kind_launches[10] = {0, 0, 0, 0, 0, 0, 0, 0, 0, 0};
    int profiled_runs = 0;
    parsy::RefineState* refine = nullptr;
    parsy::SelinvState* selinv = nullptr;
};

namespace parsy {

parsy_plan* plan_build(const PatternRef& P, const size_t* lC, const int* A2p, const int* A2i,
                       int device);
void plan_free(parsy_plan* plan);
int plan_upload_launches(parsy_plan* plan);
int plan_factor(parsy_plan* plan, const double* d_values, double* d_L, hipStream_t stream,
                bool init = true);
int plan_factor_begin(parsy_plan* plan, const double* d_values, double* d_L, hipStream_t stream, bool init);
int plan_factor_levels(parsy_plan* plan, int level0, int level1, double* d_L, hipStream_t stream);
int plan_factor_end(parsy_plan* plan, hipStream_t stream);
void plan_factor_abort(parsy_plan* plan, hipStream_t stream);
int plan_solve(parsy_plan* plan, const double* d_L, double* d_x, int nrhs, int ldx,
               hipStream_t stream);
int plan_backsolve(parsy_plan* plan, const double* d_L, double* d_x, int nrhs, int ldx, hipStream_t stream);
int plan_solve_levels(parsy_plan* plan, const double* d_L, double* d_x, int nrhs, int ldx, hipStream_t stream, int lev0,
                      int lev1, int flags);
int plan_collect_profile(parsy_plan* plan);
hipError_t grow_device(double*& buf, int64_t& len, int64_t need);

}
```

### parsy_bench_amd/csrc/kernels.hpp

```cpp
#pragma once
#include <hip/hip_runtime.h>

#include <cstdint>

#include "schedule.hpp"

namespace parsy {

constexpr int kPassLanes = 8;

struct SolveGates {
    int mrhs_min = 6;
    int chain_mrhs_min = 2;
    int bmrhs_min = 16;
    bool bmrhs_wide_only = true;
    int bchain_min_blocks = 128;
    int small_halves_min = 512;
    int sub_mrhs_min = 6;
    int xt_min = 16;
    bool xt_min_set = false;
    int wait_bias = 0;
    int sub_abl = 0;
};
SolveGates read_solve_gates();

#define PARSY_WITNESS_KERNELS(X)                                                                                     \
    X(SolveTiny, "k_solve_tiny<16>")                                                                                 \
    X(SolveSmall, "k_solve_small")                                                                                   \
    X(SolveSmallMrhs16, "k_solve_small_mrhs<16>")                                                                    \
    X(SolveSmallMrhs32, "k_solve_small_mrhs<32>")                                                                    \
    X(SolveSmallMrhs64, "k_solve_small_mrhs<64>")                                                                    \
    X(SolveSmallMrhs64Halves, "k_solve_small_mrhs<64,true>")                                                         \
    X(SolvePanel, "k_solve_panel")                                                                                   \
    X(DiagInverse, "k_diag_inverse")                                                                                 \
    X(SolveChainW2, "k_solve_chain_w<2>")                                                                            \
    X(SolveChainW4, "k_solve_chain_w<4>")                                                                            \
    X(SolveBlocksMrhsNarrow, "k_solve_blocks_mrhs<true>")                                                            \
    X(SolveBlocksMrhs, "k_solve_blocks_mrhs<false>")                                                                 \
    X(TransposeX, "k_transpose_x")                                                                                   \
    X(SolveArmWide, "k_solve_arm_wide")                                                                              \
    X(SolveOne1, "k_solve_one<1>")                                                                                   \
    X(SolveOne4, "k_solve_one<4>")                                                                                   \
    X(SolveOne8, "k_solve_one<8>")                                                                                   \
    X(BsolveOne1, "k_bsolve_one<1>")                                                                                 \
    X(BsolveOne4, "k_bsolve_one<4>")                                                                                 \
    X(BsolveOne8, "k_bsolve_one<8>")                                                                                 \
    X(BsolveBlock1, "k_bsolve_block<1>")                                                                             \
    X(BsolveBlock4, "k_bsolve_block<4>")                                                                             \
    X(BsolveBlockMrhs1, "k_bsolve_block_mrhs<1>")                                                                    \
    X(BsolveBlockMrhs4, "k_bsolve_block_mrhs<4>")                                                                    \
    X(BsolveChainMrhs, "k_bsolve_chain_mrhs")                                                                        \
    X(BsolveTiny16, "k_bsolve_tiny<16>")                                                                             \
    X(BsolveTiny32, "k_bsolve_tiny<32>")                                                                             \
    X(BsolveTinyMrhs, "k_bsolve_tiny_mrhs")                                                                          \
    X(BsolveBelow, "k_bsolve_below")                                                                                 \
    X(BsolveChainW, "k_bsolve_chain_w")                                                                              \
    X(SolveFixup, "k_solve_fixup")                                                                                   \
    X(RhsOnes, "k_rhs_ones")                                                                                         \
    X(CopySegments, "k_copy_segments")                                                                               \
    X(SolveSubMrhs, "k_solve_sub_mrhs")                                                                              \
    X(BsolveSubMrhs, "k_bsolve_sub_mrhs")
enum WitnessKernel : int {
#define PARSY_WITNESS_ENUM(id, name) kW##id,
    PARSY_WITNESS_KERNELS(PARSY_WITNESS_ENUM)
#undef PARSY_WITNESS_ENUM
    kWitnessCount
};
void witness_launch(WitnessKernel k);

struct DevicePattern {
    const SnDesc* sn = nullptr;
    const SnDesc* csn = nullptr;
    const UpdDesc* upd = nullptr;
    const int32_t* relpos = nullptr;
    const int64_t* a_dst = nullptr;
    const int32_t* rows = nullptr;
    const WaveEntry* wave_entries = nullptr;
    const int64_t* wave_ptr = nullptr;
    const int64_t* split_ranges = nullptr;
    double* tile_scratch = nullptr;
    const int32_t* small_list = nullptr;
    const int32_t* small_ranges = nullptr;
    const int32_t* solve_small_ranges = nullptr;
    const int32_t* bsolve_ranges = nullptr;
    const TileDesc* tiles = nullptr;
    const WaveEntry* big_entries = nullptr;
    const TileDesc* big_tasks = nullptr;
    const int32_t* solve_small_list = nullptr;
    const PanelDesc* solve_panels = nullptr;
    const PanelDesc* solve_mtasks = nullptr;
    const int32_t* solve_fix_list = nullptr;
    const int32_t* solve_wide_list = nullptr;
    const PanelDesc* bsolve_pairs = nullptr;
    const PanelDesc* bsolve_below = nullptr;
    double* bpart = nullptr;
    const PanelDesc* bsolve_blocks = nullptr;
    const SubMember* sub_members = nullptr;
    const SubTree* sub_trees = nullptr;
    const uint16_t* sub_slots = nullptr;
    const int32_t* sub_out_rows = nullptr;
    int sub_ntiers = 0;
    int* info = nullptr;
    int* tflags = nullptr;
    int n_tflags = 0;
    int* tickets = nullptr;
    int* sinfo = nullptr;
    int* stickets = nullptr;
    struct OneDev {
        const SnDesc* sn = nullptr;
        const int64_t* slot0 = nullptr;
        const int32_t* wleft = nullptr;
        const int32_t* pull_ptr = nullptr;
        const int32_t* pull_slot = nullptr;
        const int32_t* pull_pos = nullptr;
        int nblocks = 0;
        int64_t nslots = 1;
    } one_f, one_b;
    SolveGates gates;
};

void launch_scatter_a(const double* values, const int64_t* a_dst, double* L, int64_t nnz,
                      hipStream_t stream);
void launch_chol_small(const DevicePattern& P, int first, int count, int lds_bytes, int stage_cap, bool subtrees,
                       double* L, hipStream_t stream);
void launch_chol_big(const DevicePattern& P, int first, int count, double* L, hipStream_t stream);
void launch_chol_dense(const DevicePattern& P, int first, int count, double* L, hipStream_t stream);
void launch_chol_tiles(const DevicePattern& P, int first, int count, double* L, hipStream_t stream);
int chain_workgroups_per_cu();
void launch_chol_chain(const DevicePattern& P, int first, int count, int ticket, int epoch, bool rows, double* L,
                       hipStream_t stream);

void launch_solve_small(const DevicePattern& P, int first, int count, int wmax, bool subtrees, const double* L,
                        double* x, int nrhs, int ldx, int ldq, hipStream_t stream);
void launch_solve_one(const DevicePattern& P, const double* L, double* x, int nrhs, int ldx,
                      double* y, double* y_next, int* state, int* state_next, int wait_bias, int cap, hipStream_t stream);
void launch_bsolve_one(const DevicePattern& P, int n, const double* L, double* x, int nrhs, int ldx,
                       double* y, double* y_next, int* state, int* state_next, int wait_bias, int cap, hipStream_t stream);
void launch_solve_panel(const DevicePattern& P, int first, int count, const double* L, double* x,
                        double* xscratch, int nrhs, int ldx, hipStream_t stream);
void launch_solve_chain(const DevicePattern& P, int first, int count, const double* L, const double* dinv, double* x,
                        double* xscratch, int ticket, int wait_bias, hipStream_t stream);
void launch_solve_blocks_mrhs(const DevicePattern& P, int first, int count, const double* L, const double* dinv,
                              double* x, double* xscratch, int nrhs, int ldx, int ldq, int ticket, int wait_bias,
                              hipStream_t stream);
void launch_transpose_x(double* x, int64_t ldx, double* xt, int64_t ldq, int n, int nrhs, bool to_rows, hipStream_t stream);
void launch_solve_sub_mrhs(const DevicePattern& P, const SubTier& T, const double* L, double* x, int nrhs, int ldx, int ldq,
                           hipStream_t stream);
void launch_bsolve_sub_mrhs(const DevicePattern& P, const SubTier& T, const double* L, double* x, int nrhs, int ldx,
                            hipStream_t stream);
int solve_sub_prepare(int max_slots);
hipError_t solve_arm_handoff(double* xscratch, int64_t n, hipStream_t stream);
void launch_solve_arm_wide(const DevicePattern& P, int npairs, double* xscratch, int nrhs, int ldx, int ldq, int ntickets,
                           hipStream_t stream);
void launch_diag_inverse(const DevicePattern& P, int count, const double* L, double* dinv,
                         hipStream_t stream);
void launch_bsolve_chain_w(const DevicePattern& P, int first, int count, const double* L, const double* dinv,
                           double* x, double* xscratch, int ticket, int wait_bias, hipStream_t stream);
void launch_bsolve_below(const DevicePattern& P, int first, int count, const double* L, const double* x, hipStream_t stream);
void launch_bsolve_block(const DevicePattern& P, int first, int count, const double* L, const double* dinv,
                         double* x, double* xscratch, int nrhs, int ldx, int mode, int tiny, int ticket,
                         int wait_bias, hipStream_t stream);
void launch_rhs_ones(const DevicePattern& P, int nsuper, int max_rows, const double* L, double* b,
                     hipStream_t stream);
void launch_copy_segments(double* dst, const double* src, const int64_t* dst_off, const int64_t* src_off,
                          const int32_t* len, int64_t nseg, hipStream_t stream);
void launch_solve_fixup(const DevicePattern& P, int first, int count, double* x,
                        const double* xscratch, int nrhs, int ldx, hipStream_t stream);

}
```

### parsy_bench_amd/csrc/schedule.cpp

```cpp
#include "schedule.hpp"

#include <cstdio>
#include <map>
#include <algorithm>
#include <queue>
#include <climits>
#include <cmath>
#include <cstdlib>
#include <cstdint>
#include <functional>
#include <stdexcept>
#include <string>

namespace parsy {

static inline int ceil_div(int a, int b) { return (a + b - 1) / b; }

static int env_int(const char* name, int dflt) {
    const char* v = std::getenv(name);
    if (!v || !*v) return dflt;
    return std::atoi(v);
}

static int find_subtrees(const std::vector<int>& parent, const std::vector<uint8_t>& eligible,
                         const std::vector<double>& cost, double cap, std::vector<int32_t>& subtree,
                         const std::vector<std::pair<int32_t, int32_t>>* slots = nullptr, int64_t slot_cap = 0) {
    const int ns = (int)parent.size();
    subtree.assign(ns, -1);
    std::vector<uint8_t> whole(eligible);
    std::vector<double> sub(cost);
    std::vector<int64_t> cols(slots ? ns : 0);
    for (int s = 0; s < ns && slots; ++s) cols[s] = (*slots)[s].first;
    for (int s = 0; s < ns; ++s) {
        const int p = parent[s];
        if (p < 0) continue;
        if (p <= s) return 0;
        if (!whole[s]) whole[p] = 0;
        sub[p] += sub[s];
        if (slots) cols[p] += cols[s];
    }
    int count = 0;
    for (int s = ns - 1; s >= 0; --s) {
        const int p = parent[s];
        if (p >= 0 && subtree[p] >= 0) subtree[s] = subtree[p];
        else if (whole[s] && sub[s] <= cap && (!slots || cols[s] + (*slots)[s].second <= slot_cap)) subtree[s] = count++;
    }
    return count;
}

void build_schedule(const PatternRef& P, const size_t* lC, const int* A2p, const int* A2i,
                    const uint8_t* active, Schedule& S, int compute_units) {
    S = Schedule();
    if (compute_units > 0) S.walker_batch = std::max(4, std::min(kWalkerBatch, compute_units / 2));
    const int n = P.n, ns = P.nsuper;
    S.n = n;
    S.nsuper = ns;
    S.solve_only = (A2p == nullptr);
    S.nnzA = A2p ? A2p[n] : 0;
    S.rows.assign(P.s, P.s + P.i_ptr[n]);
    S.ssize = (int64_t)P.i_ptr[n];
    S.xsize = (int64_t)lC[n];
    S.sn.resize(ns);
    for (int t = 0; t < ns; ++t) {
        SnDesc& d = S.sn[t];
        d.c0 = P.super[t];
        d.w = P.super[t + 1] - P.super[t];
        d.r = (int)(P.i_ptr[P.super[t + 1]] - P.i_ptr[P.super[t]]);
        d.ld = d.r;
        d.rbias = 0;
        d.px = (int64_t)lC[d.c0];
        d.pi = (int64_t)P.i_ptr[d.c0];
        d.a0 = A2p ? A2p[d.c0] : 0;
        d.a1 = A2p ? A2p[P.super[t + 1]] : 0;
        d.upd0 = 0;
        d.nupd = 0;
        d.dslot = -1;
        d.tflag0 = -1;
        if (d.w <= 0 || d.r < d.w) throw std::runtime_error("schedule: malformed supernode");
        if ((int64_t)d.w * d.r > 0x7fffffffLL)
            throw std::runtime_error("schedule: a single panel exceeds 2^31 entries");
        for (int col = d.c0; col < d.c0 + d.w; ++col)
            if (lC[col + 1] - lC[col] != (size_t)d.r || P.i_ptr[col] != P.i_ptr[d.c0])
                throw std::runtime_error("schedule: lC / Li_ptr are not a column-major panel layout");
        S.max_width = std::max(S.max_width, d.w);
        S.max_rows = std::max(S.max_rows, d.r);
        S.nnzL += (int64_t)d.w * d.r - (int64_t)d.w * (d.w - 1) / 2;
        for (int k = 0; k < d.w; ++k) S.flops_stored += (double)(d.r - k) * (double)(d.r - k);
        for (int k = 0; k < d.w; ++k)
            if (S.rows[d.pi + k] != d.c0 + k)
                throw std::runtime_error("schedule: supernode rows do not start with its own columns");
        if (d.w > kTile) {
            d.dslot = (int32_t)S.n_dslots;
            S.n_dslots += ceil_div(d.w, kTile);
        }
    }

    std::vector<int64_t> uptr(ns + 1, 0);
    std::vector<int> usn, ulb, uub;
    if (!S.solve_only) build_update_lists(P, uptr, usn, ulb, uub);
    std::vector<int64_t> urel(usn.size(), 0);
    S.a_dst.assign((size_t)S.nnzA, 0);
    std::vector<int> map(n, -1), stamp(n, -1);
    for (int t = 0; t < ns; ++t) {
        const SnDesc& T = S.sn[t];
        for (int k = 0; k < T.r; ++k) {
            const int row = S.rows[T.pi + k];
            map[row] = k;
            stamp[row] = t;
        }
        for (int col = T.c0; !S.solve_only && col < T.c0 + T.w; ++col)
            for (int q = A2p[col]; q < A2p[col + 1]; ++q) {
                const int row = A2i[q];
                if (stamp[row] != t) throw std::runtime_error("schedule: A entry outside the pattern of L");
                S.a_dst[q] = (int64_t)lC[col] + map[row];
            }
        for (int64_t u = uptr[t]; u < uptr[t + 1]; ++u) {
            const SnDesc& D = S.sn[usn[u]];
            urel[u] = (int64_t)S.relpos.size();
            for (int k = ulb[u]; k < D.r; ++k) {
                const int row = S.rows[D.pi + k];
                if (stamp[row] != t)
                    throw std::runtime_error("schedule: descendant row missing from the target's pattern");
                S.relpos.push_back(map[row]);
            }
            const double K = D.w, m = D.r - ulb[u], n1 = uub[u] - ulb[u] + 1;
            S.update_flops += K * n1 * (n1 + 1) + 2.0 * K * (m - n1) * n1;
            S.reread_bytes += 8.0 * K * m;
        }
    }
    if (S.relpos.size() > 0x7fffffffULL) throw std::runtime_error("schedule: relative index array exceeds int32");
// ... 409 lines not shown
        S.big_entries.resize(bigk.size());
        const bool dense_strips = env_int("PARSY_DENSE_STRIPS", 1) != 0;
        std::map<std::pair<int64_t, int64_t>, size_t> strip_of;
        std::vector<uint8_t> absorbed;
        int t = 0;
        for (size_t i = 0; i < bigk.size();) {
            size_t j = i;
            while (j < bigk.size() && bigk[j].launch_tile == bigk[i].launch_tile) ++j;
            const int64_t launch = bigk[i].launch_tile >> 40, tile = bigk[i].launch_tile & ((1LL << 40) - 1);
            size_t at = i;
            int64_t weight = 0, dweight = 0, dchunks = 0;
            const int lmode = launch_dense[(size_t)launch];
            if (lmode)
                for (size_t q = i; q < j; ++q)
                    if (is_dense(bigk[q].e, lmode)) {
                        S.big_entries[at++] = bigk[q].e;
                        dchunks += ceil_div(bigk[q].e.K, kDenseChunk);
                        dweight += ceil_div(bigk[q].e.K, 16) + 2;
                        {
                            const WaveEntry& E = bigk[q].e;
                            const int mi = E.mn & 255, nj = (E.mn >> 8) & 255;
                            double pairs = 0;
                            for (int jj = E.ja; jj < E.ja + nj; ++jj) pairs += std::max(0, E.ia + mi - std::max(E.ia, jj));
                            S.dense_flops += 2.0 * E.K * pairs;
                        }
                    }
            const size_t mid = at;
            int32_t nstrips = 0;
            absorbed.assign(j - i, 0);
            if (lmode && dense_strips && mid > i) {
                strip_of.clear();
                for (size_t d = i; d < mid; ++d) {
                    const WaveEntry& E = S.big_entries[d];
                    if ((E.mn & 0xffff) == (kBigTile | (kBigTile << 8))) strip_of[{E.src, ((int64_t)E.ia << 32) | (uint32_t)E.ja}] = d;
                }
                for (size_t q = i; q < j && !strip_of.empty(); ++q) {
                    const WaveEntry& R = bigk[q].e;
                    if (is_dense(R, lmode)) continue;
                    const int mi = R.mn & 255, nj = (R.mn >> 8) & 255;
                    const bool row_strip = mi <= kStripMax && nj == kBigTile, col_strip = nj <= kStripMax && mi == kBigTile;
                    if (!row_strip && !col_strip) continue;
                    const auto it = strip_of.find({R.src, ((int64_t)(R.ia - (row_strip ? kBigTile : 0)) << 32) |
                                                          (uint32_t)(R.ja - (col_strip ? kBigTile : 0))});
                    if (it == strip_of.end()) continue;
                    WaveEntry& E = S.big_entries[it->second];
                    if (E.K != R.K || ((E.mn >> 16) & 1) != ((R.mn >> 16) & 1) || E.rel != R.rel || E.ld != R.ld) continue;
                    if ((row_strip ? big_strip_rows(E) : big_strip_cols(E)) != 0) continue;
                    if (big_strip_rows(E) == 0 && big_strip_cols(E) == 0) ++nstrips;
                    E.mn |= row_strip ? mi << 17 : nj << 22;
                    absorbed[q - i] = 1;
                    {
                        double pairs = 0;
                        for (int jj = R.ja; jj < R.ja + nj; ++jj) pairs += std::max(0, R.ia + mi - std::max(R.ia, jj));
                        S.dense_flops += 2.0 * R.K * pairs;
                    }
                    dweight += ceil_div(R.K, 64);
                }
            }
            for (size_t q = i; q < j; ++q)
                if (!is_dense(bigk[q].e, lmode) && !absorbed[q - i]) {
                    S.big_entries[at++] = bigk[q].e;
                    weight += ceil_div(bigk[q].e.K, 16) + 4;
                }
            const size_t jend = at;
            S.n_dense_entries += (int64_t)(mid - i);
            S.n_strip_entries += nstrips;
            while (t + 1 < nc && big_tile0[t + 1] <= tile) ++t;
            if (tile < big_tile0[t]) {
                t = 0;
                while (big_tile0[t + 1] <= tile) ++t;
            }
            const int nbr128 = ceil_div(S.csn[t].r, kBigTile);
            const int64_t local = tile - big_tile0[t];
            S.big_all.push_back(Schedule::BigTask{t, (int32_t)(local % nbr128) * kBigTile,
                                                  (int32_t)(local / nbr128) * kBigTile,
                                                  (int32_t)std::min<int64_t>(weight, INT32_MAX), (int64_t)i, (int64_t)jend,
                                                  (int32_t)(launch >> 1), (int32_t)((launch & 1) == 0), bigk[i].sr, bigk[i].sc,
                                                  (int64_t)mid, (int32_t)std::min<int64_t>(dweight, INT32_MAX),
                                                  (int32_t)std::min<int64_t>(dchunks, INT32_MAX), nstrips});
            i = j;
        }
    }

    build_launches(S, active);
}

static void build_solve_one(Schedule& S, bool sharded);

static bool append_sub_tier(Schedule& S, const std::vector<std::vector<int32_t>>& trees, int top_level, int max_slots) {
    const size_t members0 = S.sub_members.size(), trees0 = S.sub_trees.size(), slots0 = S.sub_slots.size(),
                 outs0 = S.sub_out_rows.size();
    auto drop = [&] {
        S.sub_members.resize(members0);
        S.sub_trees.resize(trees0);
        S.sub_slots.resize(slots0);
        S.sub_out_rows.resize(outs0);
        return false;
    };
    if (trees.empty()) return false;
    std::vector<int32_t> col_slot((size_t)S.n, -1);
    std::vector<int32_t> out_slot((size_t)S.n, -1);
    std::vector<int32_t> root_slot((size_t)S.nsuper, -1);
    std::vector<int32_t> owner;
    SubTier tier{(int32_t)trees0, 0, 0, top_level};
    for (const std::vector<int32_t>& tree : trees) {
        SubTree T{};
        T.m0 = (int32_t)S.sub_members.size();
        T.out0 = (int32_t)S.sub_out_rows.size();
        for (size_t q = tree.size(); q-- > 0;) {
            const int32_t t = tree[q];
            const SnDesc& D = S.sn[t];
            const int p = S.sparent[(size_t)t];
            const int32_t off = (p >= 0 && root_slot[(size_t)p] >= 0) ? root_slot[(size_t)p] + S.sn[p].w : 0;
            root_slot[(size_t)t] = off;
            for (int c = 0; c < D.w; ++c) col_slot[(size_t)D.c0 + c] = off + c;
            T.ncols = std::max(T.ncols, off + D.w);
        }
        std::vector<int32_t> outs;
        for (int32_t t : tree) {
            const SnDesc& D = S.sn[t];
            for (int k = D.w; k < D.r; ++k) {
                const int32_t row = S.rows[(size_t)D.pi + k];
                if (col_slot[(size_t)row] < 0 && out_slot[(size_t)row] < 0) {
                    out_slot[(size_t)row] = 0;
                    outs.push_back(row);
                }
            }
        }
        std::sort(outs.begin(), outs.end());
        T.nout = (int32_t)outs.size();
        for (int32_t j = 0; j < T.nout; ++j) out_slot[(size_t)outs[(size_t)j]] = T.ncols + j;
        S.sub_out_rows.insert(S.sub_out_rows.end(), outs.begin(), outs.end());
        const int32_t trash = T.ncols + T.nout;
        bool ok = trash + 1 <= max_slots && trash + 1 <= 65535;
        auto row_id = [&](const SnDesc& D, int k) { return k < D.w ? D.c0 + k : S.rows[(size_t)D.pi + k]; };
        auto slot_of = [&](int32_t row) { return col_slot[(size_t)row] >= 0 ? col_slot[(size_t)row] : out_slot[(size_t)row]; };
        for (size_t q = 0; q < tree.size() && ok; ++q) {
            const SnDesc& D = S.sn[tree[q]];
            for (int j0 = 0; j0 < D.w; j0 += kTinyWidth) {
                const int wb = std::min(kTinyWidth, D.w - j0);
                SubMember M{D.px + (int64_t)j0 * D.r + j0, D.c0 + j0, wb, D.r - j0, root_slot[(size_t)tree[q]] + j0,
                            (int32_t)(S.sub_slots.size() / 16), D.r};
                for (int k0 = wb; k0 < M.r; k0 += 16)
                    for (int kq = 0; kq < 4; ++kq)
                        for (int v = 0; v < 4; ++v) {
                            const int k = k0 + 4 * v + kq;
                            S.sub_slots.push_back((uint16_t)(k < M.r ? slot_of(row_id(D, j0 + k)) : trash));
                        }
                S.sub_members.push_back(M);
            }
        }
        T.m1 = (int32_t)S.sub_members.size();
        owner.assign((size_t)T.ncols, -1);
        for (size_t q = 0; q < tree.size() && ok; ++q) {
            const SnDesc& D = S.sn[tree[q]];
            for (int c = 0; c < D.w && ok; ++c) {
                int32_t& o = owner[(size_t)col_slot[(size_t)D.c0 + c]];
                ok = o < 0 || o == D.c0 + c;
                o = -1;
            }
            for (int k = D.w; k < D.r && ok; ++k) {
                const int32_t row = S.rows[(size_t)D.pi + k];
                if (col_slot[(size_t)row] < 0) continue;
                int32_t& o = owner[(size_t)col_slot[(size_t)row]];
                ok = o < 0 || o == row;
                o = row;
// ... 206 lines not shown
            std::vector<Group> groups;
            for (const auto& kb : keyed) {
                if (groups.empty() || groups.back().key != kb.first) groups.push_back(Group{kb.first, 0, 0, {}});
                Group& G = groups.back();
                G.tasks.push_back(kb.second);
                G.weight += wt(kb.second);
                G.maxw = std::max(G.maxw, wt(kb.second));
            }
            std::stable_sort(groups.begin(), groups.end(), [](const Group& a, const Group& b) {
                return a.maxw != b.maxw ? a.maxw > b.maxw : a.weight > b.weight;
            });
            const size_t bulk = groups.size() > (size_t)kBigTailGroups ? groups.size() - kBigTailGroups : 0;
            rest.clear();
            for (size_t q = 0; q < groups.size(); ++q) {
                Group& G = groups[q];
                if (q >= bulk) {
                    rest.insert(rest.end(), G.tasks.begin(), G.tasks.end());
                    continue;
                }
                const int x = least();
                std::stable_sort(G.tasks.begin(), G.tasks.end(), by_weight);
                seq[x].insert(seq[x].end(), G.tasks.begin(), G.tasks.end());
                load[x] += G.weight;
            }
        }
        size_t len = 0;
        for (int x = 0; x < 8; ++x) len = std::max(len, seq[x].size());
        for (size_t s = 0; s < len; ++s)
            for (int x = 0; x < 8; ++x) {
                if (s < seq[x].size()) {
                    S.big_tasks.push_back(desc(seq[x][s]));
                } else {
                    S.big_tasks.push_back(TileDesc{0, 0, 0, 0, 0, 0});
                }
            }
        L.count = (int32_t)(8 * len);
        return L;
    };
    auto subtree_ranges = [&](const std::vector<int32_t>& subtree, int count, const std::vector<double>& cost,
                              auto&& position, auto&& append, std::vector<int32_t>& ranges, bool chol = false) {
        std::vector<std::vector<int32_t>> members((size_t)count);
        std::vector<double> total((size_t)count, 0.0);
        for (int t = 0; t < ns; ++t)
            if (subtree[t] >= 0 && (chol ? S.active_piece[S.piece0[t]] : S.active[t])) {
                members[(size_t)subtree[t]].push_back(t);
                total[(size_t)subtree[t]] += cost[t];
            }
        std::vector<int32_t> order;
        for (int k = 0; k < count; ++k)
            if (!members[(size_t)k].empty()) order.push_back(k);
        std::stable_sort(order.begin(), order.end(), [&](int a, int b) { return total[(size_t)a] > total[(size_t)b]; });
        for (int k : order) {
            ranges.push_back(position());
            for (int32_t t : members[(size_t)k]) append(t);
            ranges.push_back(position());
        }
        return (int32_t)order.size();
    };
    S.small_ranges.clear();
    S.solve_small_ranges.clear();
    S.bsolve_ranges.clear();
    S.sub_members.clear();
    S.sub_trees.clear();
    S.sub_slots.clear();
    S.sub_out_rows.clear();
    S.sub_max_slots = 0;
    S.bsolve_blocks.clear();
    S.bsolve_pairs.clear();
    for (int lev = 0; lev < S.cnlevels && !S.solve_only; ++lev) {
        level_begin.push_back(S.chol.size());
        bigs.clear();
        if (lev == 0 && S.n_chol_subtrees > 0) {
            Launch L{kLaunchSmall, 0, 0, 0, 0, 0, 2, 0, -1, 0};
            L.count = subtree_ranges(
                S.chol_subtree, S.n_chol_subtrees, S.chol_cost, [&] { return (int32_t)S.small_list.size(); },
                [&](int32_t t) {
                    const SnDesc& T = S.csn[S.piece0[t]];
                    S.small_list.push_back(S.piece0[t]);
                    L.lds_bytes = std::max<int32_t>(L.lds_bytes, T.w * T.r * (int)sizeof(double));
                    for (int64_t u = T.upd0; u < T.upd0 + T.nupd; ++u)
                        L.jb = std::max<int32_t>(L.jb, std::min<int64_t>((int64_t)S.upd[u].m * S.upd[u].K, 2048));
                },
                S.small_ranges, true);
            if (L.count > 0) S.chol.push_back(L);
        }
        {
            Launch L{kLaunchSmall, (int32_t)S.small_list.size(), 0, lev, 0, 0, 0, 0, -1, 0};
            for (int q = S.clevelPtr[lev]; q < S.clevelPtr[lev + 1]; ++q) {
                const int t = S.clevelSet[q];
                if (!S.active_piece[t] || S.chol_subtree[S.csn_real[t]] >= 0) continue;
                const SnDesc& T = S.csn[t];
                if (is_small(T)) {
                    S.small_list.push_back(t);
                    L.lds_bytes = std::max<int32_t>(L.lds_bytes, T.w * T.r * (int)sizeof(double));
                    for (int64_t u = T.upd0; u < T.upd0 + T.nupd; ++u)
                        L.jb = std::max<int32_t>(L.jb, std::min<int64_t>((int64_t)S.upd[u].m * S.upd[u].K, 2048));
                } else {
                    bigs.push_back(t);
                }
            }
            L.count = (int32_t)S.small_list.size() - L.first;
            if (L.count > 0) S.chol.push_back(L);
        }
        if (lev + 2 < S.cnlevels) {
            Launch Ld = emit_big(big_push[lev], Launch{kLaunchDense, 0, 0, lev + 2, 0, 0, 0, 1, lev, 1}, true);
            if (Ld.count > 0) early_launches.push_back(Ld);
            Launch Lp = emit_big(big_push[lev], Launch{kLaunchBig, 0, 0, lev + 2, 0, 0, 0, 1, lev, 1}, false);
            if (Lp.count > 0) early_launches.push_back(Lp);
        }
        if (lev > 0) {
            Launch Ld = emit_big(big_next[lev - 1], Launch{kLaunchDense, 0, 0, lev, 0, 0, 0, 0, -1, 0}, true);
            if (Ld.count > 0) S.chol.push_back(Ld);
            Launch Ln = emit_big(big_next[lev - 1], Launch{kLaunchBig, 0, 0, lev, 0, 0, 0, 0, -1, 0}, false);
            if (Ln.count > 0) S.chol.push_back(Ln);
        }
        if (!bigs.empty()) {
            {
                Launch Lt{kLaunchTiles, (int32_t)S.tiles.size(), 0, lev, 0, 0, 0, 1, lev - 2, 1};
                std::vector<std::pair<int32_t, TileDesc>> wt;
                for (int t : bigs) {
                    const SnDesc& T = S.csn[t];
                    const int nbc = ceil_div(T.w, kTile), nbr = ceil_div(T.r, kTile);
                    const int32_t* tw = &S.tile_w[S.sn_tw0[t]];
                    for (int J = 0; J < nbc; ++J)
                        for (int I = J; I < nbr; ++I) {
                            const int32_t wgt = tw[((size_t)J * nbr + I) * 2];
                            if (wgt <= 0) continue;
                            const int64_t si = S.tile_split[S.sn_tw0[t] / 2 + (size_t)J * nbr + I];
                            if (si < 0) {
                                wt.push_back({wgt, TileDesc{t, I * kTile, J * kTile, 0,
                                                            S.sn_wp0[t] + (((int64_t)J * nbr + I) * 2) * 4, -1}});
                            } else {
                                const Schedule::SplitDesc& sd = S.split_desc[(size_t)si];
                                for (int part = 0; part < sd.nparts; ++part)
                                    wt.push_back({ceil_div(wgt, sd.nparts),
                                                  TileDesc{t, I * kTile, J * kTile, part | (sd.nparts << 8),
                                                           sd.ranges + part * 8, sd.sp}});
                            }
                        }
                }
                std::stable_sort(wt.begin(), wt.end(),
                                 [](const auto& a, const auto& b) { return a.first > b.first; });
                for (auto& x : wt) S.tiles.push_back(x.second);
                Lt.count = (int32_t)S.tiles.size() - Lt.first;
                if (Lt.count > 0) early_launches.push_back(Lt);
            }
            const int chain_split_mode = env_int("PARSY_CHAIN_SPLIT", S.update_flops >= kChainSplitAutoFlops ? 2 : 0);
            auto splits = [&](int t) {
                const int real = S.csn_real[t];
                return chain_split_mode == 2 || (chain_split_mode == 1 && S.piece0[real + 1] - S.piece0[real] > 1);
            };
            bool chain_split = false;
            for (int t : bigs) chain_split = chain_split || splits(t);
            for (int part = 0; part < (chain_split ? 2 : 1); ++part) {
            Launch Lc{kLaunchChain, (int32_t)S.tiles.size(), 0, lev, S.n_chain_launches++, 0, 0, 0, -1, 0};
            Lc.fused = part;
            for (size_t b0 = 0; b0 < bigs.size(); b0 += (size_t)S.walker_batch) {
              const size_t b1 = std::min(bigs.size(), b0 + (size_t)S.walker_batch);
              int maxnb = 0;
              for (size_t q = b0; q < b1; ++q) maxnb = std::max(maxnb, ceil_div(S.csn[bigs[q]].w, kTile));
              for (int J = 0; J < maxnb; ++J)
                for (size_t q = b0; q < b1; ++q) {
                    const int t = bigs[q];
                    const SnDesc& T = S.csn[t];
                    const int nbc = ceil_div(T.w, kTile), nbr = ceil_div(T.r, kTile);
                    if (J >= nbc) continue;
                    auto push = [&](int I, int Jc) {
                        if (chain_split && ((I < nbc || !splits(t)) != (part == 0))) return;
                        const int64_t si = S.tile_split[S.sn_tw0[t] / 2 + (size_t)Jc * nbr + I];
                        S.tiles.push_back(TileDesc{t, I * kTile, Jc * kTile,
                                                   si < 0 ? 0 : S.split_desc[(size_t)si].nparts,
                                                   S.sn_wp0[t] + (((int64_t)Jc * nbr + I) * 2 + 1) * 4,
                                                   si < 0 ? -1 : S.split_desc[(size_t)si].sp});
                    };
                    if (J == 0) push(0, 0);
                    const bool next_diag = J + 1 < nbc;
                    if (next_diag) {
                        push(J + 1, J);
                        push(J + 1, J + 1);
                    }
                    for (int I = next_diag ? J + 2 : J + 1; I < nbr; ++I) push(I, J);
                }
            }
            Lc.count = (int32_t)S.tiles.size() - Lc.first;
// ... 650 lines not shown
}

template <class Fail>
static void check_sub_tiers(const Schedule& S, Fail&& fail) {
    if (S.sub_tiers.empty()) return;
    const int ns = S.nsuper;
    std::vector<int32_t> sn_of_col((size_t)S.n, -1);
    for (int t = 0; t < ns; ++t)
        for (int c = 0; c < S.sn[t].w; ++c) sn_of_col[(size_t)S.sn[t].c0 + c] = t;
    std::vector<int> level((size_t)ns, 0);
    for (int l = 0; l < S.nlevels; ++l)
        for (int q = S.levelPtr[l]; q < S.levelPtr[l + 1]; ++q) level[(size_t)S.levelSet[q]] = l;
    std::vector<int32_t> tree_of((size_t)ns, -1);
    int32_t next_tree = 0;
    for (size_t k = 0; k < S.sub_tiers.size(); ++k) {
        const SubTier& R = S.sub_tiers[k];
        if (R.tree0 != next_tree || R.ntrees <= 0 || (size_t)(R.tree0 + R.ntrees) > S.sub_trees.size())
            return fail("sub tiers: tiers do not tile the trees");
        next_tree = R.tree0 + R.ntrees;
        if (k == 0 && (size_t)R.ntrees != S.solve_small_ranges.size() / 2) return fail("sub tiers: tier 0 is not the subtree launch");
        for (int32_t b = R.tree0; b < R.tree0 + R.ntrees; ++b) {
            const SubTree& T = S.sub_trees[(size_t)b];
            if (T.m0 >= T.m1 || (size_t)T.m1 > S.sub_members.size() || T.ncols + T.nout + 1 > R.max_slots ||
                (size_t)(T.out0 + T.nout) > S.sub_out_rows.size())
                return fail("sub tiers: a tree's ranges");
            int32_t prev_sn = -1, expect_c = -1;
            for (int32_t q = T.m0; q < T.m1; ++q) {
                const SubMember& M = S.sub_members[(size_t)q];
                if (M.c0 < 0 || M.c0 >= S.n || M.w < 1 || M.w > kTinyWidth) return fail("sub tiers: a member's columns");
                const int t = sn_of_col[(size_t)M.c0];
                const SnDesc& D = S.sn[t];
                const int j0 = M.c0 - D.c0;
                if (!S.active[t] || j0 % kTinyWidth != 0 || M.w != std::min(kTinyWidth, D.w - j0) || M.r != D.r - j0 || M.ld != D.r ||
                    M.px != D.px + (int64_t)j0 * D.r + j0)
                    return fail("sub tiers: a member is not a 16-column block of an active supernode");
                if (j0 == 0) {
                    if (tree_of[(size_t)t] >= 0) return fail("sub tiers: a supernode in two trees");
                    if (t <= prev_sn) return fail("sub tiers: members out of index order");
                    if (k == 0 ? S.solve_subtree[t] < 0 : (level[(size_t)t] > R.top_level || S.sn[t].w > kSubTierMaxWidth))
                        return fail("sub tiers: a supernode that does not belong to its tier");
                    tree_of[(size_t)t] = b;
                    prev_sn = t;
                } else if (t != prev_sn || M.c0 != expect_c) {
                    return fail("sub tiers: the blocks of a supernode are not in a row");
                }
                expect_c = M.c0 + M.w;
                if (M.slot0 < 0 || M.slot0 + M.w > T.ncols) return fail("sub tiers: a member's column slots");
                const int nch = (M.r - M.w + 15) / 16;
                if ((size_t)(M.so + nch) * 16 > S.sub_slots.size()) return fail("sub tiers: a member's slot words");
                for (int ch = 0; ch < nch; ++ch)
                    for (int e = 0; e < 16; ++e) {
                        const int k2 = M.w + 16 * ch + 4 * (e & 3) + (e >> 2), slot = S.sub_slots[(size_t)(M.so + ch) * 16 + e];
                        if (k2 >= M.r) {
                            if (slot != T.ncols + T.nout) return fail("sub tiers: a padding row not in the padding slot");
                            continue;
                        }
                        const int32_t row = j0 + k2 < D.w ? D.c0 + j0 + k2 : S.rows[(size_t)D.pi + j0 + k2];
                        if (slot < T.ncols) {
                            const int tt = sn_of_col[(size_t)row];
                            bool found = false;
                            for (int32_t q2 = q + 1; q2 < T.m1 && !found; ++q2) {
                                const SubMember& M2 = S.sub_members[(size_t)q2];
                                found = row >= M2.c0 && row < M2.c0 + M2.w && slot == M2.slot0 + row - M2.c0;
                            }
                            if (!found || tt < 0) return fail("sub tiers: a row's column slot does not belong to a later member");
                        } else if (slot >= T.ncols + T.nout || S.sub_out_rows[(size_t)T.out0 + slot - T.ncols] != row) {
                            return fail("sub tiers: a row's outside slot");
                        }
                    }
            }
            for (int32_t j = 0; j < T.nout; ++j) {
                const int32_t row = S.sub_out_rows[(size_t)T.out0 + j];
                if (j > 0 && row <= S.sub_out_rows[(size_t)T.out0 + j - 1]) return fail("sub tiers: outside rows not sorted");
                if (tree_of[(size_t)sn_of_col[(size_t)row]] == b) return fail("sub tiers: an outside row is a column of the tree");
            }
        }
    }
    for (int t = 0; t < ns; ++t) {
        if (S.solve_subtree[t] >= 0 && S.active[t] && tree_of[(size_t)t] < 0) return fail("sub tiers: a supernode of the subtree launch is missing");
        if (S.active[t] && level[(size_t)t] <= S.sub_cover_level && tree_of[(size_t)t] < 0) return fail("sub tiers: a covered level has a supernode outside the tiers");
    }
}

int64_t check_schedule(const Schedule& S, std::string& what) {
    int64_t bad = 0;
    auto fail = [&](const std::string& msg) {
        if (bad++ == 0) what = msg;
    };
    check_solve_launches(S, fail);
    check_solve_one(S, fail);
    check_sub_tiers(S, fail);
    if (S.solve_only) return bad;
    const int nc = (int)S.csn.size();
    for (int t = 0; t < S.nsuper; ++t) {
        int cols = 0;
        for (int p = S.piece0[t]; p < S.piece0[t + 1]; ++p) {
            const SnDesc& C = S.csn[p];
            if (C.c0 != S.sn[t].c0 + cols || C.rbias != cols || C.r != S.sn[t].r - cols || C.ld != S.sn[t].r)
                fail("piece " + std::to_string(p) + " is not a window of its supernode's panel");
            if (p > S.piece0[t] && S.level_of[p] != S.level_of[p - 1] + 1) fail("pieces of a supernode are not on consecutive levels");
            cols += C.w;
        }
        if (cols != S.sn[t].w) fail("pieces of supernode " + std::to_string(t) + " do not add up to its width");
    }
    std::vector<double> covered(S.upd.size(), 0.0);
    auto entry_flops = [](const WaveEntry& E, bool same_window) {
        const double K = E.K, mi = E.mn & 255, nj = (E.mn >> 8) & 255;
        return same_window ? K * nj * (nj + 1) + 2.0 * K * (mi - nj) * nj : 2.0 * K * mi * nj;
    };
    auto block_flops = [](const WaveEntry& E) {
        const int mi = E.mn & 255, nj = (E.mn >> 8) & 255;
        auto pairs_of = [](int ia, int m, int ja, int n) {
            double pairs = 0;
            for (int j = ja; j < ja + n; ++j) pairs += std::max(0, ia + m - std::max(ia, j));
            return pairs;
        };
        return 2.0 * E.K * (pairs_of(E.ia, mi, E.ja, nj) + pairs_of(E.ia + mi, big_strip_rows(E), E.ja, nj) +
                            pairs_of(E.ia, mi, E.ja + nj, big_strip_cols(E)));
    };
    for (int t = 0; t < nc; ++t) {
        const SnDesc& T = S.csn[t];
        for (int64_t u = T.upd0; u < T.upd0 + T.nupd; ++u)
            if (S.level_of[S.upd_src[u]] >= S.level_of[t]) fail("update " + std::to_string(u) + " comes from a level that is not below its target");
        if (is_small(T) || T.nupd == 0) continue;
        auto find_upd = [&](const WaveEntry& E) -> int64_t {
            for (int64_t u = T.upd0; u < T.upd0 + T.nupd; ++u)
                if (S.upd[u].src == E.src && S.upd[u].K == E.K) return u;
            return -1;
        };
        if (S.sn_wp0[t] >= 0) {
            const int nbc = ceil_div(T.w, kTile), nbr = ceil_div(T.r, kTile);
            const int64_t* wp = &S.wave_ptr[S.sn_wp0[t]];
            for (size_t key = 0; key < (size_t)nbc * nbr * 8; ++key)
                for (int64_t e = wp[key]; e < wp[key + 1]; ++e) {
                    const WaveEntry& E = S.wave_entries[(size_t)e];
                    const int64_t u = find_upd(E);
                    const int mi = E.mn & 255, nj = (E.mn >> 8) & 255;
                    if (u < 0 || mi < 1 || mi > kSub || nj < 1 || nj > kSub || E.ia + mi > S.upd[u].m || E.ja + nj > S.upd[u].n1) {
                        fail("wave entry " + std::to_string(e) + " of piece " + std::to_string(t) + " has a bad window");
                        continue;
                    }
                    covered[(size_t)u] += entry_flops(E, E.ia == E.ja);
                }
        }
    }
    for (const Schedule::BigTask& b : S.big_all) {
        const SnDesc& T = S.csn[b.sn];
        if (b.src_level >= S.level_of[b.sn] || (b.next != 0) != (b.src_level == S.level_of[b.sn] - 1))
            fail("BIG task of piece " + std::to_string(b.sn) + " is filed under the wrong source level");
        const int win_r = kBigTile * b.sr, win_c = kBigTile * b.sc;
        if (b.sr < 1 || b.sc < 1 || b.row0 % win_r || b.col0 % win_c || b.row0 + win_r <= b.col0 || b.row0 >= T.r || b.col0 >= T.w)
            fail("BIG task of piece " + std::to_string(b.sn) + " has a bad tile origin");
        for (int64_t e = b.e0; e < b.e1; ++e) {
            const WaveEntry& E = S.big_entries[(size_t)e];
            int64_t u = -1;
            for (int64_t q = T.upd0; q < T.upd0 + T.nupd; ++q)
                if (S.upd[q].src == E.src && S.upd[q].K == E.K) u = q;
            const int mi = E.mn & 255, nj = (E.mn >> 8) & 255;
            const bool ident = big_ident(E);
            const int ms = big_strip_rows(E), ns = big_strip_cols(E);
            if ((ms || ns) && (e >= b.em || mi != kBigTile || nj != kBigTile || ms > kStripMax || ns > kStripMax))
                fail("BIG entry " + std::to_string(e) + " carries a strip but is not a full dense block");
            if (u < 0 || mi < 1 || mi > kBigTile || nj < 1 || nj > kBigTile || E.ia + mi + ms > S.upd[u].m || E.ja + nj + ns > S.upd[u].n1 ||
                ident != (S.upd[u].rel < 0) || S.level_of[S.upd_src[u]] != b.src_level) {
                fail("BIG entry " + std::to_string(e) + " of piece " + std::to_string(b.sn) + " has a bad window or source");
                continue;
// ... 45 lines not shown
        }
        std::sort(starts.begin(), starts.end());
        if (std::adjacent_find(starts.begin(), starts.end()) != starts.end()) fail("a BIG task is launched twice");
        int64_t want = 0;
        for (size_t k = 0; k < S.big_all.size(); ++k) {
            const Schedule::BigTask& b = S.big_all[k];
            if (b.em < b.e0 || b.em > b.e1) fail("BIG task " + std::to_string(k) + " has a bad dense / ragged split");
            int64_t dch = 0;
            int32_t nst = 0;
            for (int64_t e = b.e0; e < b.em; ++e) {
                const WaveEntry& E = S.big_entries[(size_t)e];
                nst += big_strip_rows(E) || big_strip_cols(E);
                if (E.K < kDenseChunk) fail("BIG entry " + std::to_string(e) + " is filed as dense but is narrower than a chunk");
                dch += ceil_div(E.K, kDenseChunk);
            }
            if (dch != b.dchunks) fail("BIG task " + std::to_string(k) + " has a wrong dense chunk count");
            if (nst != b.strips) fail("BIG task " + std::to_string(k) + " has a wrong count of entries with strips");
            if (!S.active_piece[b.sn]) continue;
            want += (b.em > b.e0) + (b.e1 > b.em);
            if (b.em > b.e0 && b.e1 > b.em && !(dense_pos[k] > 0 && ragged_pos[k] > dense_pos[k]))
                fail("BIG task " + std::to_string(k) + ": the ragged part is not launched after the dense part");
        }
        if ((int64_t)starts.size() != want)
            fail("BIG launches hold " + std::to_string(starts.size()) + " task parts, the active targets have " + std::to_string(want));
    }
    for (int t = 0; t < nc; ++t) {
        const SnDesc& T = S.csn[t];
        if (is_small(T)) continue;
        for (int64_t u = T.upd0; u < T.upd0 + T.nupd; ++u) {
            const UpdDesc& U = S.upd[u];
            const double want = (double)U.K * U.n1 * (U.n1 + 1) + 2.0 * U.K * (double)(U.m - U.n1) * U.n1;
            if (std::abs(covered[(size_t)u] - want) > 1e-9 * want + 0.5)
                fail("update " + std::to_string(u) + " of piece " + std::to_string(t) + " is not covered exactly once by its entries");
        }
    }
    for (int t = 0; t < nc; ++t) {
        const int real = S.csn_real[t], st = S.chol_subtree[real];
        if (st < 0) continue;
        if (!is_small(S.csn[t])) fail("supernode " + std::to_string(real) + " of a subtree is not a SMALL one");
        for (int64_t u = S.csn[t].upd0; u < S.csn[t].upd0 + S.csn[t].nupd; ++u)
            if (S.chol_subtree[S.csn_real[S.upd_src[u]]] != st)
                fail("supernode " + std::to_string(real) + " of a subtree is updated from outside the subtree");
    }
    {
        std::vector<int> seen(nc, 0);
        for (const Launch& l : S.chol) {
            if (l.kind != kLaunchSmall) continue;
            if (l.fused == 2) {
                for (int b = l.first; b < l.first + l.count; ++b) {
                    const int32_t q0 = S.small_ranges[2 * (size_t)b], q1 = S.small_ranges[2 * (size_t)b + 1];
                    if (q0 < 0 || q1 <= q0 || q1 > (int32_t)S.small_list.size()) {
                        fail("subtree launch: bad range " + std::to_string(b));
                        continue;
                    }
                    for (int32_t q = q0; q < q1; ++q) {
                        seen[S.small_list[q]]++;
                        if (q > q0 && S.small_list[q] <= S.small_list[q - 1]) fail("subtree launch: a run is not in index order");
                        if (S.chol_subtree[S.csn_real[S.small_list[q]]] != S.chol_subtree[S.csn_real[S.small_list[q0]]])
                            fail("subtree launch: a run mixes subtrees");
                    }
                }
            } else {
                for (int q = l.first; q < l.first + l.count; ++q) seen[S.small_list[q]]++;
            }
        }
        for (int t = 0; t < nc; ++t)
            if (seen[t] != ((is_small(S.csn[t]) && S.active_piece[t]) ? 1 : 0))
                fail("SMALL supernode " + std::to_string(t) + " is in " + std::to_string(seen[t]) + " launches");
    }
    int main_level = -1;
    for (size_t i = 0; i < S.chol.size(); ++i) {
        const Launch& l = S.chol[i];
        if (l.side) {
            if (l.wait_level >= 0 && main_level > l.wait_level + 0 && main_level >= l.level)
                fail("side launch " + std::to_string(i) + " is enqueued after the level that waits for it");
            for (size_t j = i + 1; j < S.chol.size(); ++j)
                if (!S.chol[j].side && S.chol[j].level <= l.wait_level)
                    fail("side launch " + std::to_string(i) + " precedes a main-stream launch of a level it waits for");
        } else {
            if (l.level < main_level) fail("main-stream launches go down a level");
            main_level = l.level;
        }
    }
    return bad;
}

}
```

### parsy_bench_amd/csrc/schedule.hpp

```cpp
#pragma once
#include <cstddef>
#include <cstdint>
#include <string>
#include <vector>

#include "inspector.hpp"

namespace parsy {

constexpr int kTile = 64;
constexpr int kSub = 32;
constexpr int kSmallMaxEntries = 6144;
constexpr int kSmallMaxWidth = 64;
constexpr int kBelowRows = 512;
constexpr int kBelowMaxGroups = 512;
constexpr int kBackGroup = 2;
constexpr int kTinyWidth = 16;
constexpr int kTinyWidth2 = 32;
constexpr int kPanelRows = 128;
constexpr int kSolveRows = 256;
constexpr int kSolveRowsMrhs = 128;

struct SnDesc {
    int64_t px;
    int64_t pi;
    int64_t upd0;
    int32_t c0, w, r;
    int32_t nupd;
    int32_t a0, a1;
    int32_t dslot;
    int32_t tflag0;
    int32_t ld;
    int32_t rbias;
};

struct UpdDesc {
    int64_t src;
    int64_t rel;
    int32_t ld;
    int32_t K;
    int32_t m;
    int32_t n1;
};

struct WaveEntry {
    int64_t src;
    int32_t rel;
    int32_t ld, K;
    int32_t ia, ja;
    int32_t mn;
};
constexpr int kStripMax = 16;
inline bool big_ident(const WaveEntry& E) { return (E.mn >> 16) & 1; }
inline int big_strip_rows(const WaveEntry& E) { return (E.mn >> 17) & 31; }
inline int big_strip_cols(const WaveEntry& E) { return (E.mn >> 22) & 31; }
constexpr int kDenseStripTask = 1 << 30;

struct TileDesc {
    int32_t sn;
    int32_t row0, col0;
    int32_t part;
    int64_t wp;
    int64_t sp;
};

struct PanelDesc {
    int32_t sn;
    int32_t jb;
    int32_t row0;
    int32_t pad;
};

struct SubMember {
    int64_t px;
    int32_t c0, w, r;
    int32_t slot0;
    int32_t so;
    int32_t ld;
};
struct SubTree {
    int32_t m0, m1;
    int32_t ncols;
    int32_t nout;
    int32_t out0;
    int32_t pad[3];
};
struct SubTier {
    int32_t tree0, ntrees;
    int32_t max_slots;
    int32_t top_level;
};
constexpr int kSubMaxSlots = 320;
constexpr int kSubTierMaxWidth = 64;
constexpr int kSubTierMinTrees = 512;
constexpr int kSubTierMaxSlots = 448;
constexpr int kSubTierMaxDensity = 700;

enum LaunchKind : int32_t {
    kLaunchSmall = 0, kLaunchTiles = 1, kLaunchChain = 2, kLaunchBig = 3,
    kLaunchBackBelow = 4,
    kLaunchSolveSmall = 5, kLaunchSolvePanel = 6, kLaunchSolveFixup = 7, kLaunchBackBlock = 8,
    kLaunchDense = 9,
};
inline bool is_chol_launch(int kind) { return (kind >= 0 && kind <= kLaunchBig) || kind == kLaunchDense; }

struct Launch {
    int32_t kind;
    int32_t first, count;
    int32_t level;
    int32_t jb;
    int32_t lds_bytes;
    int32_t fused;
    int32_t side;
    int32_t wait_level;
    int32_t early;
};

constexpr int kSplitChunks = 192;
constexpr int kSplitTarget = 128;
constexpr int kSplitMaxParts = 4;
constexpr int kSplitFewTiles = 128;
constexpr int kSplitFewChunks = 32;
constexpr int kSplitFewTarget = 24;
constexpr int kSplitFewMaxParts = 8;
constexpr int kWalkerBatch = 64;
constexpr int kBigTile = 128;
constexpr int kBigMinK = 128;
constexpr int kPieceWidth = 512;
constexpr double kBigAutoFlops = 1e11;
constexpr double kPieceAutoFlops = 2e12;
constexpr double kChainSplitAutoFlops = 1e11;
constexpr int kBigSuperMinTasks = 12288;
constexpr double kBigSuperMaxFill = 0.85;
constexpr int kBigGroup = 8;
constexpr int kBigGroupsPerXcd = 2;
constexpr int kBigTailGroups = 16;
constexpr int kDenseChunk = 8;
constexpr double kDenseMinShare = 0.25;
constexpr double kDenseMinFill = 0.70;
constexpr double kDenseAllShare = 0.06;
constexpr int kPushGroup = 1;
constexpr int kOneMaxSupernodes = 8192;
constexpr int64_t kOneLargeEntries = 4096;
constexpr int64_t kOneMaxEntries = 1 << 28;
constexpr int kOneMaxSupernodesBig = 32768;
constexpr int kOneSmallBlocks = 1024;
constexpr int kOneMidBlocks = 4096;
constexpr int kOneRhs8Density = 300;
constexpr int kOneMaxRhs = 8;
constexpr int kCholSubtreesPerCu = 64;
constexpr int kSubtreesPerCu = 16;
constexpr double kSubtreeMinCost = 2e5;
constexpr int kSubtreeMinPerSlot = 2;
constexpr int kSolveSubtreeMinMembers = 2048;

struct Schedule {
    int n = 0, nsuper = 0, nlevels = 0;
    bool solve_only = false;
    int64_t nnzA = 0, ssize = 0, xsize = 0, nnzL = 0;
    int max_width = 0, max_rows = 0, n_small = 0, n_big = 0;
    int n_solve_wide = 0;
    int64_t n_dslots = 0;
    int64_t n_tflags = 0;
    int n_chain_launches = 0;
    int n_solve_chain_launches = 0;
    int walker_batch = kWalkerBatch;
    double flops_stored = 0, update_flops = 0, reread_bytes = 0;
    double tile_update_flops = 0;
    double inner_flops = 0;

    std::vector<SnDesc> sn;
    std::vector<int> sparent;
    std::vector<SnDesc> csn;
    std::vector<int32_t> piece0;
    std::vector<int32_t> csn_real;
    std::vector<int> clevelPtr, clevelSet;
    int cnlevels = 0;
    int big_min_k = kBigMinK, piece_width = kPieceWidth, push_group = kPushGroup;
    int big_super_r = 0, big_super_c = 0;
    std::vector<UpdDesc> upd;
    std::vector<int32_t> upd_src;
    std::vector<int32_t> relpos;
    std::vector<int64_t> a_dst;
    std::vector<int32_t> rows;
    std::vector<WaveEntry> wave_entries;
    std::vector<int64_t> wave_ptr;

    std::vector<int32_t> chol_subtree, solve_subtree, bsolve_subtree;
    std::vector<int32_t> solve_subtree_all, bsolve_subtree_all;
    std::vector<double> chol_cost, solve_cost;
    int n_chol_subtrees = 0, n_solve_subtrees = 0, n_bsolve_subtrees = 0;
    std::vector<int32_t> small_ranges, solve_small_ranges, bsolve_ranges;
    std::vector<SubMember> sub_members;
    std::vector<SubTree> sub_trees;
    std::vector<uint16_t> sub_slots;
    std::vector<int32_t> sub_out_rows;
    std::vector<SubTier> sub_tiers;
    int sub_cover_level = -1;
    int sub_max_slots = 0;

    std::vector<int32_t> small_list;
    std::vector<TileDesc> tiles;
    std::vector<WaveEntry> big_entries;
    struct BigTask { int32_t sn, row0, col0, weight; int64_t e0, e1; int32_t src_level, next;
                     int32_t sr, sc;
                     int64_t em; int32_t dweight, dchunks;
                     int32_t strips; };
    std::vector<BigTask> big_all;
    std::vector<TileDesc> big_tasks;
    double big_flops = 0;
    double dense_flops = 0;
    int64_t n_dense_entries = 0;
    int64_t n_strip_entries = 0;
    std::vector<Launch> chol;

    std::vector<int32_t> solve_small_list;
    std::vector<PanelDesc> solve_panels;
    std::vector<PanelDesc> solve_mtasks;
    std::vector<int32_t> solve_fix_list;
    std::vector<int32_t> solve_wide_list;
    std::vector<Launch> solve;

    std::vector<PanelDesc> bsolve_pairs;
    std::vector<PanelDesc> bsolve_blocks;
    std::vector<PanelDesc> bsolve_below;
    int64_t n_bpart_slots = 0;
    std::vector<Launch> bsolve;

    struct OneLists {
        std::vector<SnDesc> sn;
        std::vector<int64_t> slot0;
        std::vector<int32_t> wleft;
        int64_t nslots = 0;
        std::vector<int32_t> pull_ptr, pull_slot, pull_pos;
        std::vector<uint8_t> member;
        void clear() { *this = OneLists(); }
    };
    bool solve_one = false, solve_one_back = false;
    bool one_subtrees = false;
    bool one_big = false;
    bool one_forced = false;
    OneLists one_f, one_b;
    const OneLists& one_back() const { return one_b.sn.empty() ? one_f : one_b; }

    std::vector<uint8_t> active;
    std::vector<uint8_t> active_piece;
    std::vector<size_t> chol_level_begin;
    std::vector<int> levelPtr, levelSet;
    std::vector<int64_t> split_ranges;
    std::vector<int64_t> tile_split;
    struct SplitDesc { int64_t ranges; int64_t sp; int32_t nparts; int32_t pad; };
    std::vector<SplitDesc> split_desc;
    int64_t n_split_doubles = 0;
    std::vector<int64_t> sn_wp0;
    std::vector<int64_t> sn_tw0;
    std::vector<int32_t> tile_w;
    std::vector<int32_t> level_of;
};

void build_schedule(const PatternRef& P, const size_t* lC, const int* A2p, const int* A2i,
                    const uint8_t* active, Schedule& out, int compute_units = 0);
void build_launches(Schedule& S, const uint8_t* active, const uint8_t* active_pieces = nullptr);
int64_t simulate_chain(const Schedule& S, int slots);
int64_t check_schedule(const Schedule& S, std::string& what);
constexpr int kSmallMaxUpdates = 8;
inline bool is_small(const SnDesc& d) {
    return d.w <= kSmallMaxWidth && (int64_t)d.w * d.r <= kSmallMaxEntries && d.nupd <= kSmallMaxUpdates;
}

}
```

Measured before the change: 2.976 factorizations/s.

## Split L initialisation and overlap deferred zero-fill with early small-supernode launches

Supernodes whose panels and update sources are all small single-piece ones are marked early. Only their panels are zeroed and scattered from A on the main stream before the first small launches. The remaining panels (the large bulk of xsize) are zero-filled and scattered on a separate init stream with a limited group count, and main and side launches wait on an init event before touching them. This hides the large memset of roughly 2.4G doubles behind leaf factorization work. It adds range-based fill and scatter kernels, extra events and streams, and competition for bandwidth with concurrent kernels.

```diff
diff --git a/include/parsy_amd.h b/include/parsy_amd.h
--- a/include/parsy_amd.h
+++ b/include/parsy_amd.h
@@ -82,6 +82,9 @@
     int32_t sub_mrhs_tiers;
     int32_t sub_mrhs_cover_level;
     int64_t dense_strip_entries;
+    int64_t init_early_entries, init_deferred_entries;
+    int32_t init_ranges;
+    int32_t init_split;
 } parsy_plan_info;
 
 parsy_plan* parsy_plan_create(int n, int supNo, const int* blockSet, const size_t* lC,
@@ -177,7 +180,7 @@
 double parsy_last_factor_ms(parsy_plan* plan);
 double parsy_last_solve_ms(parsy_plan* plan);
 
-#define PARSY_PROFILE_KINDS 10
+#define PARSY_PROFILE_KINDS 11
 int parsy_plan_profile(parsy_plan* plan, int enable);
 int parsy_plan_profile_collect(parsy_plan* plan);
 int parsy_plan_profile_get(parsy_plan* plan, double* kind_ms, int* kind_launches, int* runs);
diff --git a/parsy_bench_amd/_native.py b/parsy_bench_amd/_native.py
--- a/parsy_bench_amd/_native.py
+++ b/parsy_bench_amd/_native.py
@@ -54,6 +54,8 @@
         ("sub_mrhs_trees", C.c_int32), ("sub_mrhs_slots", C.c_int32),
         ("sub_mrhs_tiers", C.c_int32), ("sub_mrhs_cover_level", C.c_int32),
         ("dense_strip_entries", C.c_int64),
+        ("init_early_entries", C.c_int64), ("init_deferred_entries", C.c_int64),
+        ("init_ranges", C.c_int32), ("init_split", C.c_int32),
     ]
 
     def as_dict(self):
diff --git a/parsy_bench_amd/api.py b/parsy_bench_amd/api.py
--- a/parsy_bench_amd/api.py
+++ b/parsy_bench_amd/api.py
@@ -6,7 +6,8 @@
 
 from . import _native as N
 
-KIND_NAMES = ["SMALL", "TILES", "CHAIN", "BIG", "BACK_BELOW", "SOLVE_SMALL", "SOLVE_PANEL", "SOLVE_FIXUP", "BACK_BLOCK", "DENSE"]
+KIND_NAMES = ["SMALL", "TILES", "CHAIN", "BIG", "BACK_BELOW", "SOLVE_SMALL", "SOLVE_PANEL", "SOLVE_FIXUP", "BACK_BLOCK", "DENSE",
+              "INIT"]
 
 
 def device_count() -> int:
@@ -349,8 +350,8 @@
             raise RuntimeError("profile_collect: no profiled run to collect")
 
     def profile_get(self) -> dict:
-        ms = np.zeros(10, dtype=np.float64)
-        cnt = np.zeros(10, dtype=np.int32)
+        ms = np.zeros(len(KIND_NAMES), dtype=np.float64)
+        cnt = np.zeros(len(KIND_NAMES), dtype=np.int32)
         runs = C.c_int(0)
         N.lib().parsy_plan_profile_get(self._h, N.ptr(ms), N.ptr(cnt), C.byref(runs))
         return {"runs": runs.value, "ms": dict(zip(KIND_NAMES, ms.tolist())),
diff --git a/parsy_bench_amd/csrc/capi_exec.hip b/parsy_bench_amd/csrc/capi_exec.hip
--- a/parsy_bench_amd/csrc/capi_exec.hip
+++ b/parsy_bench_amd/csrc/capi_exec.hip
@@ -336,6 +336,10 @@
     o->sub_mrhs_tiers = (int32_t)S.sub_tiers.size();
     o->sub_mrhs_cover_level = S.sub_cover_level;
     o->dense_strip_entries = S.n_strip_entries;
+    o->init_early_entries = S.init_set[0].entries();
+    o->init_deferred_entries = S.init_set[1].entries();
+    o->init_ranges = (int32_t)(S.init_set[0].l_off.size() + S.init_set[1].l_off.size());
+    o->init_split = S.init_split ? 1 : 0;
     return 0;
 }
 
@@ -566,7 +570,7 @@
     if (!pl) return -1;
     pl->profile = enable != 0;
     if (enable == 2) {
-        for (int k = 0; k < 10; ++k) pl->kind_ms[k] = 0, pl->kind_launches[k] = 0;
+        for (int k = 0; k < parsy::kProfileKinds; ++k) pl->kind_ms[k] = 0, pl->kind_launches[k] = 0;
         pl->profiled_runs = 0;
         pl->level_ms.clear();
     }
@@ -577,7 +581,7 @@
 
 int parsy_plan_profile_get(parsy_plan* pl, double* kind_ms, int* kind_launches, int* runs) {
     if (!pl) return -1;
-    for (int k = 0; k < 10; ++k) {
+    for (int k = 0; k < parsy::kProfileKinds; ++k) {
         if (kind_ms) kind_ms[k] = pl->kind_ms[k];
         if (kind_launches) kind_launches[k] = pl->kind_launches[k];
     }
diff --git a/parsy_bench_amd/csrc/chol_kernels.hip b/parsy_bench_amd/csrc/chol_kernels.hip
--- a/parsy_bench_amd/csrc/chol_kernels.hip
+++ b/parsy_bench_amd/csrc/chol_kernels.hip
@@ -52,6 +52,84 @@
     if (blocks > 4096) blocks = 4096;
     hipLaunchKernelGGL(k_scatter_a, dim3((unsigned)blocks), dim3(kThreads), 0, stream, values, a_dst,
                        L, nnz);
+}
+
+static constexpr int kFillChunk = 65536;
+static constexpr int kScatterChunk = 4096;
+static constexpr int kInitMaxGroups = 2048;
+
+__device__ static inline int range_of(const int64_t* __restrict__ pre, int nranges, int64_t p) {
+    int lo = 0, hi = nranges;
+    while (hi - lo > 1) {
+        const int mid = (lo + hi) >> 1;
+        if (pre[mid] <= p) lo = mid;
+        else hi = mid;
+    }
+    return lo;
+}
+
+__global__ __launch_bounds__(kThreads) void k_fill_ranges(const int64_t* __restrict__ off, const int64_t* __restrict__ pre,
+                                                          int nranges, double* __restrict__ L) {
+    typedef double double2_t __attribute__((ext_vector_type(2)));
+    const int64_t total = pre[nranges];
+    for (int64_t c0 = (int64_t)blockIdx.x * kFillChunk; c0 < total; c0 += (int64_t)gridDim.x * kFillChunk) {
+        const int64_t c1 = c0 + kFillChunk < total ? c0 + kFillChunk : total;
+        int i = range_of(pre, nranges, c0);
+        for (int64_t p = c0; p < c1; ++i) {
+            const int64_t e = pre[i + 1] < c1 ? pre[i + 1] : c1;
+            double* dst = L + off[i] + (p - pre[i]);
+            int64_t len = e - p;
+            p = e;
+            if (len <= 0) continue;
+            int64_t head = (int64_t)((16 - ((reinterpret_cast<uintptr_t>(dst) >> 3) & 15)) & 15);
+            if (head > len) head = len;
+            if ((int64_t)threadIdx.x < head) dst[threadIdx.x] = 0.0;
+            dst += head;
+            len -= head;
+            double2_t* d2 = reinterpret_cast<double2_t*>(dst);
+            const double2_t zero = {0.0, 0.0};
+            const int64_t pairs = len >> 1;
+            for (int64_t k = threadIdx.x; k < pairs; k += kThreads) d2[k] = zero;
+            if ((len & 1) && threadIdx.x == 0) dst[len - 1] = 0.0;
+        }
+    }
+}
+
+__global__ __launch_bounds__(kThreads) void k_scatter_a_ranges(const double* __restrict__ values,
+                                                               const int64_t* __restrict__ a_dst,
+                                                               const int64_t* __restrict__ off,
+                                                               const int64_t* __restrict__ pre, int nranges,
+                                                               double* __restrict__ L) {
+    const int64_t total = pre[nranges];
+    for (int64_t c0 = (int64_t)blockIdx.x * kScatterChunk; c0 < total; c0 += (int64_t)gridDim.x * kScatterChunk) {
+        const int64_t c1 = c0 + kScatterChunk < total ? c0 + kScatterChunk : total;
+        int i = range_of(pre, nranges, c0);
+        for (int64_t p = c0; p < c1; ++i) {
+            const int64_t e = pre[i + 1] < c1 ? pre[i + 1] : c1;
+            const int64_t q0 = off[i] + (p - pre[i]), len = e - p;
+            p = e;
+            for (int64_t k = threadIdx.x; k < len; k += kThreads) L[a_dst[q0 + k]] = values[q0 + k];
+        }
+    }
+}
+
+static unsigned init_groups(int64_t total, int chunk, int max_groups = kInitMaxGroups) {
+    const int64_t chunks = (total + chunk - 1) / chunk;
+    return (unsigned)(chunks < max_groups ? chunks : max_groups);
+}
+
+void launch_fill_ranges(const int64_t* off, const int64_t* pre, int nranges, int64_t total, double* L, int max_groups,
+                        hipStream_t stream) {
+    if (total <= 0 || nranges <= 0) return;
+    hipLaunchKernelGGL(k_fill_ranges, dim3(init_groups(total, kFillChunk, max_groups > 0 ? max_groups : kInitMaxGroups)),
+                       dim3(kThreads), 0, stream, off, pre, nranges, L);
+}
+
+void launch_scatter_a_ranges(const double* values, const int64_t* a_dst, const int64_t* off, const int64_t* pre,
+                             int nranges, int64_t total, double* L, hipStream_t stream) {
+    if (total <= 0 || nranges <= 0) return;
+    hipLaunchKernelGGL(k_scatter_a_ranges, dim3(init_groups(total, kScatterChunk)), dim3(kThreads), 0, stream, values, a_dst,
+                       off, pre, nranges, L);
 }
 
 typedef double double2_t __attribute__((ext_vector_type(2)));
diff --git a/parsy_bench_amd/csrc/executor.hip b/parsy_bench_amd/csrc/executor.hip
--- a/parsy_bench_amd/csrc/executor.hip
+++ b/parsy_bench_amd/csrc/executor.hip
@@ -113,6 +113,13 @@
     if (upload(pl, S.upd, pl->dp.upd, false)) return -1;
     if (upload(pl, S.relpos, pl->dp.relpos, false)) return -1;
     if (upload(pl, S.a_dst, pl->dp.a_dst, false)) return -1;
+    for (int k = 0; k < 2; ++k) {
+        const Schedule::InitSet& I = S.init_set[k];
+        DevicePattern::InitDev& D = pl->dp.init_set[k];
+        if (upload(pl, I.l_off, D.l_off, false) || upload(pl, I.l_pre, D.l_pre, false) || upload(pl, I.a_off, D.a_off, false) ||
+            upload(pl, I.a_pre, D.a_pre, false))
+            return -1;
+    }
     if (upload(pl, S.rows, pl->dp.rows, false)) return -1;
     if (upload(pl, S.wave_entries, pl->dp.wave_entries, false)) return -1;
     if (upload(pl, S.wave_ptr, pl->dp.wave_ptr, false)) return -1;
@@ -148,7 +155,9 @@
         PARSY_HIP(hipDeviceGetStreamPriorityRange(&prio_least, &prio_greatest));
         PARSY_HIP(hipStreamCreateWithPriority(&pl->side_stream, hipStreamNonBlocking, prio_least));
     }
+    PARSY_HIP(hipStreamCreateWithFlags(&pl->init_stream, hipStreamNonBlocking));
     PARSY_HIP(hipEventCreateWithFlags(&pl->ev_init, hipEventDisableTiming));
+    PARSY_HIP(hipEventCreateWithFlags(&pl->ev_begin, hipEventDisableTiming));
     pl->ev_level_done.resize(std::max(S.nlevels, S.cnlevels) + 1);
     pl->ev_early_done.resize(std::max(S.nlevels, S.cnlevels) + 1);
     for (auto& e : pl->ev_level_done) PARSY_HIP(hipEventCreateWithFlags(&e, hipEventDisableTiming));
@@ -156,6 +165,10 @@
     {
         const char* no = std::getenv("PARSY_NO_OVERLAP");
         pl->overlap = !(no && no[0] == '1');
+        const char* io = std::getenv("PARSY_INIT_OVERLAP");
+        pl->init_overlap = (io && io[0] >= '0' && io[0] <= '2' && !io[1]) ? io[0] - '0' : 1;
+        const char* fg = std::getenv("PARSY_INIT_FILL_GROUPS");
+        pl->init_fill_groups = fg && std::atoi(fg) > 0 ? std::atoi(fg) : kInitBesideGroups;
     }
     PARSY_HIP(hipEventCreate(&pl->ev_f0));
     PARSY_HIP(hipEventCreate(&pl->ev_f1));
@@ -215,6 +228,8 @@
         for (hipEvent_t e : pl->ev_level_done) (void)hipEventDestroy(e);
         for (hipEvent_t e : pl->ev_early_done) (void)hipEventDestroy(e);
         if (pl->ev_init) (void)hipEventDestroy(pl->ev_init);
+        if (pl->ev_begin) (void)hipEventDestroy(pl->ev_begin);
+        if (pl->init_stream) (void)hipStreamDestroy(pl->init_stream);
         if (pl->side_stream) (void)hipStreamDestroy(pl->side_stream);
         if (pl->h_stream) (void)hipStreamDestroy(pl->h_stream);
         if (pl->h_copy) (void)hipStreamDestroy(pl->h_copy);
@@ -267,6 +282,14 @@
     for (size_t li = i0; li < i1; ++li) {
         const Launch& l = seq[li];
         const bool on_side = overlap && l.side;
+        if (!on_side && pl->init_wait_main && !is_head_launch(l)) {
+            (void)hipStreamWaitEvent(stream, pl->ev_init, 0);
+            pl->init_wait_main = false;
+        }
+        if (on_side && pl->init_wait_side) {
+            (void)hipStreamWaitEvent(pl->side_stream, pl->ev_init, 0);
+            pl->init_wait_side = false;
+        }
         if (!on_side) {
             if (overlap && is_chol_launch(l.kind)) record_levels_below(l.level);
             if (overlap && (l.kind == kLaunchChain || l.kind == kLaunchBig || l.kind == kLaunchDense)) {
@@ -547,7 +570,7 @@
         const int k = pl->pev_kind[i];
         if (pl->pev_ms.size() <= i) pl->pev_ms.resize(i + 1, 0.f);
         pl->pev_ms[i] = ms;
-        if (k >= 0 && k < 10) {
+        if (k >= 0 && k < kProfileKinds) {
             pl->kind_ms[k] += ms;
             pl->kind_launches[k] += 1;
         }
@@ -561,6 +584,13 @@
     return 0;
 }
 
+static void init_part(parsy_plan* pl, int k, const double* d_values, double* d_L, hipStream_t stream) {
+    const Schedule::InitSet& I = pl->S.init_set[k];
+    const DevicePattern::InitDev& D = pl->dp.init_set[k];
+    launch_fill_ranges(D.l_off, D.l_pre, (int)I.l_off.size(), I.entries(), d_L, k == 1 ? pl->init_fill_groups : 0, stream);
+    launch_scatter_a_ranges(d_values, pl->dp.a_dst, D.a_off, D.a_pre, (int)I.a_off.size(), I.a_entries(), d_L, stream);
+}
+
 int plan_factor_begin(parsy_plan* pl, const double* d_values, double* d_L, hipStream_t stream, bool init) {
     if (pl->device < 0) {
         set_last_error("parsy_factor: plan was built without a device (device < 0)");
@@ -576,13 +606,25 @@
         pl->epoch = 0;
     }
     pl->epoch += 1;
+    run_begin(pl);
     PARSY_HIP(hipEventRecord(pl->ev_f0, stream));
-    if (init) PARSY_HIP(hipMemsetAsync(d_L, 0, (size_t)S.xsize * sizeof(double), stream));
+    const bool split = init && pl->overlap && !pl->profile && pl->side_stream != nullptr && pl->init_stream != nullptr &&
+                       S.init_set[1].entries() > 0 && (pl->init_overlap == 2 || (pl->init_overlap == 1 && S.init_split));
+    if (init) profile_mark(pl, kProfileInit, stream, pl->run_cursor);
+    if (init && !split) PARSY_HIP(hipMemsetAsync(d_L, 0, (size_t)S.xsize * sizeof(double), stream));
     PARSY_HIP(hipMemsetAsync(pl->dp.info, 0x7f, sizeof(int), stream));
     PARSY_HIP(hipMemsetAsync(pl->dp.tickets, 0, (size_t)std::max(S.n_chain_launches, 1) * sizeof(int), stream));
-    if (init) launch_scatter_a(d_values, pl->dp.a_dst, d_L, S.nnzA, stream);
-    PARSY_HIP(hipEventRecord(pl->ev_init, stream));
-    run_begin(pl);
+    if (init && !split) launch_scatter_a(d_values, pl->dp.a_dst, d_L, S.nnzA, stream);
+    if (split) {
+        init_part(pl, 0, d_values, d_L, stream);
+        PARSY_HIP(hipEventRecord(pl->ev_begin, stream));
+        PARSY_HIP(hipStreamWaitEvent(pl->init_stream, pl->ev_begin, 0));
+        init_part(pl, 1, d_values, d_L, pl->init_stream);
+        PARSY_HIP(hipEventRecord(pl->ev_init, pl->init_stream));
+    } else {
+        PARSY_HIP(hipEventRecord(pl->ev_init, stream));
+    }
+    pl->init_wait_main = pl->init_wait_side = split;
     pl->factor_open = true;
     pl->factor_next_level = 0;
     return 0;
@@ -601,6 +643,10 @@
     if (level1 > level0)
         run_range(pl, S.chol, S.chol_level_begin[(size_t)level0], S.chol_level_begin[(size_t)level1], d_L, d_L, nullptr,
                   0, 0, stream);
+    if (pl->init_wait_main && level1 < S.cnlevels) {
+        (void)hipStreamWaitEvent(stream, pl->ev_init, 0);
+        pl->init_wait_main = false;
+    }
     profile_mark(pl, -1, stream, pl->run_cursor);
     pl->factor_next_level = level1;
     PARSY_HIP(hipGetLastError());
@@ -617,6 +663,8 @@
         return -1;
     }
     run_end(pl, stream);
+    if (pl->init_wait_main) (void)hipStreamWaitEvent(stream, pl->ev_init, 0);
+    pl->init_wait_main = pl->init_wait_side = false;
     if (pl->overlap && !pl->profile && pl->side_stream != nullptr) {
         for (size_t k = pl->run_early_seen.size(); k-- > 0;)
             if (pl->run_early_seen[k]) {
@@ -635,6 +683,8 @@
     if (!pl) return;
     (void)hipStreamSynchronize(stream);
     if (pl->side_stream != nullptr) (void)hipStreamSynchronize(pl->side_stream);
+    if (pl->init_stream != nullptr) (void)hipStreamSynchronize(pl->init_stream);
+    pl->init_wait_main = pl->init_wait_side = false;
     (void)hipGetLastError();
     if (pl->factor_open) run_end(pl, stream);
     pl->factor_open = false;
diff --git a/parsy_bench_amd/csrc/executor.hpp b/parsy_bench_amd/csrc/executor.hpp
--- a/parsy_bench_amd/csrc/executor.hpp
+++ b/parsy_bench_amd/csrc/executor.hpp
@@ -51,6 +51,11 @@
 
     hipStream_t side_stream = nullptr;
     hipEvent_t ev_init = nullptr;
+    hipStream_t init_stream = nullptr;
+    hipEvent_t ev_begin = nullptr;
+    int init_overlap = 1;
+    int init_fill_groups = parsy::kInitBesideGroups;
+    bool init_wait_main = false, init_wait_side = false;
     std::vector<hipEvent_t> ev_level_done, ev_early_done;
     bool overlap = true;
 
@@ -73,8 +78,8 @@
     std::vector<int> pev_count;
     std::vector<float> pev_ms;
     std::vector<double> level_ms;
-    double kind_ms[10] = {0, 0, 0, 0, 0, 0, 0, 0, 0, 0};
-    int kind_launches[10] = {0, 0, 0, 0, 0, 0, 0, 0, 0, 0};
+    double kind_ms[parsy::kProfileKinds] = {};
+    int kind_launches[parsy::kProfileKinds] = {};
     int profiled_runs = 0;
     parsy::RefineState* refine = nullptr;
     parsy::SelinvState* selinv = nullptr;
diff --git a/parsy_bench_amd/csrc/kernels.hpp b/parsy_bench_amd/csrc/kernels.hpp
--- a/parsy_bench_amd/csrc/kernels.hpp
+++ b/parsy_bench_amd/csrc/kernels.hpp
@@ -74,6 +74,9 @@
     const UpdDesc* upd = nullptr;
     const int32_t* relpos = nullptr;
     const int64_t* a_dst = nullptr;
+    struct InitDev {
+        const int64_t *l_off = nullptr, *l_pre = nullptr, *a_off = nullptr, *a_pre = nullptr;
+    } init_set[2];
     const int32_t* rows = nullptr;
     const WaveEntry* wave_entries = nullptr;
     const int64_t* wave_ptr = nullptr;
@@ -121,6 +124,11 @@
 
 void launch_scatter_a(const double* values, const int64_t* a_dst, double* L, int64_t nnz,
                       hipStream_t stream);
+constexpr int kInitBesideGroups = 96;
+void launch_fill_ranges(const int64_t* off, const int64_t* pre, int nranges, int64_t total, double* L, int max_groups,
+                        hipStream_t stream);
+void launch_scatter_a_ranges(const double* values, const int64_t* a_dst, const int64_t* off, const int64_t* pre,
+                             int nranges, int64_t total, double* L, hipStream_t stream);
 void launch_chol_small(const DevicePattern& P, int first, int count, int lds_bytes, int stage_cap, bool subtrees,
                        double* L, hipStream_t stream);
 void launch_chol_big(const DevicePattern& P, int first, int count, double* L, hipStream_t stream);
diff --git a/parsy_bench_amd/csrc/schedule.cpp b/parsy_bench_amd/csrc/schedule.cpp
--- a/parsy_bench_amd/csrc/schedule.cpp
+++ b/parsy_bench_amd/csrc/schedule.cpp
@@ -46,6 +46,39 @@
         else if (whole[s] && sub[s] <= cap && (!slots || cols[s] + (*slots)[s].second <= slot_cap)) subtree[s] = count++;
     }
     return count;
+}
+
+static void build_init_split(Schedule& S) {
+    for (Schedule::InitSet& I : S.init_set) {
+        I = Schedule::InitSet();
+        I.l_pre.push_back(0);
+        I.a_pre.push_back(0);
+    }
+    S.init_early.assign((size_t)S.nsuper, 0);
+    S.init_split = false;
+    if (S.solve_only) return;
+    for (int t = 0; t < S.nsuper; ++t) {
+        const int p = S.piece0[t];
+        const bool one_piece = S.piece0[t + 1] - p == 1;
+        bool early = one_piece && is_small(S.csn[p]);
+        for (int64_t u = S.csn[p].upd0; early && u < S.csn[p].upd0 + S.csn[p].nupd; ++u)
+            early = S.init_early[(size_t)S.csn_real[(size_t)S.upd_src[(size_t)u]]] != 0;
+        S.init_early[(size_t)t] = early;
+    }
+    for (int t = 0; t < S.nsuper; ++t) {
+        const SnDesc& T = S.sn[t];
+        Schedule::InitSet& I = S.init_set[S.init_early[(size_t)t] ? 0 : 1];
+        const bool joins = t > 0 && S.init_early[(size_t)t] == S.init_early[(size_t)t - 1];
+        if (!joins) {
+            I.l_off.push_back(T.px);
+            I.l_pre.push_back(I.l_pre.back());
+            I.a_off.push_back(T.a0);
+            I.a_pre.push_back(I.a_pre.back());
+        }
+        I.l_pre.back() += (int64_t)T.w * T.r;
+        I.a_pre.back() += T.a1 - T.a0;
+    }
+    S.init_split = S.init_set[1].entries() >= kInitSplitMinEntries;
 }
 
 void build_schedule(const PatternRef& P, const size_t* lC, const int* A2p, const int* A2i,
@@ -621,6 +654,7 @@
         }
     }
 
+    build_init_split(S);
     build_launches(S, active);
 }
 
@@ -993,6 +1027,8 @@
                         L.jb = std::max<int32_t>(L.jb, std::min<int64_t>((int64_t)S.upd[u].m * S.upd[u].K, 2048));
                 },
                 S.small_ranges, true);
+            L.head = 1;
+            for (int32_t t : S.small_list) L.head = L.head && S.init_early[(size_t)S.csn_real[(size_t)t]];
             if (L.count > 0) S.chol.push_back(L);
         }
         {
@@ -1011,6 +1047,8 @@
                 }
             }
             L.count = (int32_t)S.small_list.size() - L.first;
+            L.head = 1;
+            for (int q = L.first; q < L.first + L.count; ++q) L.head = L.head && S.init_early[(size_t)S.csn_real[(size_t)S.small_list[(size_t)q]]];
             if (L.count > 0) S.chol.push_back(L);
         }
         if (lev + 2 < S.cnlevels) {
@@ -1827,6 +1865,76 @@
     }
 }
 
+static void check_init_split(const Schedule& S, const std::function<void(const std::string&)>& fail) {
+    struct Range { int64_t b, e; int part; };
+    auto tiles = [&](bool a, int64_t total, std::vector<Range>& all) {
+        const char* what = a ? "A" : "lValues";
+        for (int k = 0; k < 2; ++k) {
+            const Schedule::InitSet& I = S.init_set[k];
+            const std::vector<int64_t>&off = a ? I.a_off : I.l_off, &pre = a ? I.a_pre : I.l_pre;
+            if (pre.size() != off.size() + 1 || pre[0] != 0 || I.a_off.size() != I.l_off.size()) {
+                fail(std::string("initialisation: malformed range list of ") + what);
+                return false;
+            }
+            for (size_t i = 0; i < off.size(); ++i) {
+                if (pre[i + 1] < pre[i]) fail(std::string("initialisation: prefix sums of ") + what + " ranges go down");
+                all.push_back(Range{off[i], off[i] + pre[i + 1] - pre[i], k});
+            }
+        }
+        std::stable_sort(all.begin(), all.end(), [](const Range& x, const Range& y) { return x.b < y.b; });
+        int64_t at = 0;
+        for (const Range& r : all) {
+            if (r.b != at) fail(std::string("initialisation: ") + what + " ranges leave a gap or overlap at " + std::to_string(at));
+            at = std::max(at, r.e);
+        }
+        if (at != total) fail(std::string("initialisation: ") + what + " ranges end at " + std::to_string(at) + ", not " + std::to_string(total));
+        return true;
+    };
+    std::vector<Range> lr, ar;
+    if (!tiles(false, S.xsize, lr) || !tiles(true, S.nnzA, ar)) return;
+    if ((int)S.init_early.size() != S.nsuper) {
+        fail("initialisation: no part per supernode");
+        return;
+    }
+    if (S.init_set[0].entries() + S.init_set[1].entries() != S.xsize) fail("initialisation: the parts do not add up to xsize");
+    size_t il = 0, ia = 0;
+    for (int t = 0; t < S.nsuper; ++t) {
+        const SnDesc& T = S.sn[t];
+        const int part = S.init_early[(size_t)t] ? 0 : 1;
+        const int64_t pe = T.px + (int64_t)T.w * T.r;
+        while (il < lr.size() && lr[il].e <= T.px) ++il;
+        if (il == lr.size() || lr[il].b > T.px || lr[il].e < pe || lr[il].part != part)
+            fail("initialisation: the panel of supernode " + std::to_string(t) + " is not in a range of its part");
+        if (T.a1 > T.a0) {
+            while (ia < ar.size() && ar[ia].e <= T.a0) ++ia;
+            if (ia == ar.size() || ar[ia].b > T.a0 || ar[ia].e < T.a1 || ar[ia].part != part)
+                fail("initialisation: the A entries of supernode " + std::to_string(t) + " are not in a range of its part");
+        }
+        for (int64_t q = T.a0; q < T.a1; ++q)
+            if (S.a_dst[(size_t)q] < T.px || S.a_dst[(size_t)q] >= pe) {
+                fail("initialisation: A entry " + std::to_string(q) + " lands outside its supernode's panel");
+                break;
+            }
+    }
+    auto early_piece = [&](int p) { return S.init_early[(size_t)S.csn_real[(size_t)p]] != 0; };
+    auto check_piece = [&](int p, size_t li) {
+        const SnDesc& T = S.csn[(size_t)p];
+        bool ok = early_piece(p);
+        for (int64_t u = T.upd0; ok && u < T.upd0 + T.nupd; ++u) ok = early_piece(S.upd_src[(size_t)u]);
+        if (!ok) fail("initialisation: head launch " + std::to_string(li) + " touches a deferred panel (piece " + std::to_string(p) + ")");
+    };
+    for (size_t li = 0; li < S.chol.size(); ++li) {
+        const Launch& l = S.chol[li];
+        if (!is_head_launch(l)) continue;
+        if (l.fused == 2) {
+            for (int b = l.first; b < l.first + l.count; ++b)
+                for (int q = S.small_ranges[2 * (size_t)b]; q < S.small_ranges[2 * (size_t)b + 1]; ++q) check_piece(S.small_list[(size_t)q], li);
+        } else {
+            for (int q = l.first; q < l.first + l.count; ++q) check_piece(S.small_list[(size_t)q], li);
+        }
+    }
+}
+
 int64_t check_schedule(const Schedule& S, std::string& what) {
     int64_t bad = 0;
     auto fail = [&](const std::string& msg) {
@@ -2038,6 +2146,7 @@
             main_level = l.level;
         }
     }
+    check_init_split(S, fail);
     return bad;
 }
 
diff --git a/parsy_bench_amd/csrc/schedule.hpp b/parsy_bench_amd/csrc/schedule.hpp
--- a/parsy_bench_amd/csrc/schedule.hpp
+++ b/parsy_bench_amd/csrc/schedule.hpp
@@ -103,6 +103,8 @@
     kLaunchDense = 9,
 };
 inline bool is_chol_launch(int kind) { return (kind >= 0 && kind <= kLaunchBig) || kind == kLaunchDense; }
+constexpr int kProfileInit = 10;
+constexpr int kProfileKinds = 11;
 
 struct Launch {
     int32_t kind;
@@ -114,7 +116,11 @@
     int32_t side;
     int32_t wait_level;
     int32_t early;
-};
+    int32_t head;
+};
+
+inline bool is_head_launch(const Launch& l) { return l.kind == kLaunchSmall && !l.side && l.head != 0; }
+constexpr int64_t kInitSplitMinEntries = 125000000;
 
 constexpr int kSplitChunks = 192;
 constexpr int kSplitTarget = 128;
@@ -243,6 +249,15 @@
     OneLists one_f, one_b;
     const OneLists& one_back() const { return one_b.sn.empty() ? one_f : one_b; }
 
+    struct InitSet {
+        std::vector<int64_t> l_off, l_pre, a_off, a_pre;
+        int64_t entries() const { return l_pre.empty() ? 0 : l_pre.back(); }
+        int64_t a_entries() const { return a_pre.empty() ? 0 : a_pre.back(); }
+    };
+    InitSet init_set[2];
+    std::vector<uint8_t> init_early;
+    bool init_split = false;
+
     std::vector<uint8_t> active;
     std::vector<uint8_t> active_piece;
     std::vector<size_t> chol_level_begin;
```

Result: no change. 2.986 factorizations/s (median of 6 runs) (+0.3%).
